# ipilter/RayTracerTest

Measured on AMD Instinct MI355X. Metric: Mray/s at 1920x1080x16spp, higher is better.
Workload: dtype f32

## Files before the change

### include/rt_mi355x.h

```cpp
#ifndef RT_MI355X_H
#define RT_MI355X_H

#include <stddef.h>
#include <stdint.h>

#ifdef __cplusplus
extern "C" {
#endif

#define RT_OK              0
#define RT_ERR_INVALID     1
#define RT_ERR_NO_DEVICE   2
#define RT_ERR_HIP         3
#define RT_ERR_STATE       4

#define RT_MATH_FMA        0u
#define RT_MATH_STRICT     1u

#define RT_FLAG_NO_FILTER  1u
#define RT_FLAG_NO_BINNING 2u

#define RT_FLAG_NEAREST_HIT 4u

#define RT_FLAG_NO_MACRO_BINS 16u
// ... 44 lines not shown
void rt_tracer_stop(rt_tracer* t);
int  rt_tracer_resize(rt_tracer* t, const uint32_t size[2]);
void rt_tracer_set_camera_parameters(rt_tracer* t, float fov, float focalLength, float aperture);
void rt_tracer_rotate_camera(rt_tracer* t, const float angles[2]);
int  rt_tracer_upload_scene(rt_tracer* t, const rt_float4* hostData, size_t count);
int  rt_tracer_upload_scene_edges(rt_tracer* t, const rt_float4* hostData, size_t count);
float rt_pack_normal(const float n[3]);
void  rt_unpack_normal(float packed, float n[3]);
void rt_tracer_set_update_callback(rt_tracer* t, rt_callback_fn fn, void* user);
void rt_tracer_set_finished_callback(rt_tracer* t, rt_callback_fn fn, void* user);


int  rt_tracer_wait(rt_tracer* t);
int  rt_tracer_set_seed(rt_tracer* t, uint64_t seed);
int  rt_tracer_upload_spheres(rt_tracer* t, const rt_float4* spheres, size_t count);
int  rt_tracer_trace_enqueue(rt_tracer* t, uint32_t iterationCount, uint32_t samplesPerIteration);
int  rt_tracer_trace_enqueue_n(rt_tracer* t, uint32_t iterationCount, uint32_t samplesPerIteration, uint32_t n_steps);
int  rt_tracer_sync(rt_tracer* t);
int  rt_tracer_launch(rt_tracer* t, uint32_t samples, int clear_first, int emit_image);
int  rt_tracer_launch_iterations(rt_tracer* t, uint32_t samples, uint32_t iterations, int clear_first, int emit_image);
int  rt_tracer_fused_iterations(rt_tracer* t, uint32_t samples);
int  rt_tracer_set_list_reuse(rt_tracer* t, int across_traces);
int  rt_tracer_set_image_mirror(rt_tracer* t, void* device_visible_image);
int  rt_tracer_kernel_time(rt_tracer* t, double* total_ms, uint64_t* launches, int reset_after);
int  rt_tracer_launch_time(rt_tracer* t, double* total_ms, uint64_t* launches, int reset_after);
int  rt_tracer_trace_stats(rt_tracer* t, uint32_t samples, uint64_t out[16]);
int  rt_tracer_read_buffer(rt_tracer* t, int which, void* dst, size_t bytes);
int  rt_tracer_copy_buffer_to_device(rt_tracer* t, int which, void* dst_device, size_t bytes);
int  rt_tracer_copy_buffer_to_device_async(rt_tracer* t, int which, void* dst_device, size_t bytes);
void* rt_tracer_stream(rt_tracer* t);
void* rt_tracer_stream_b(rt_tracer* t);
void* rt_tracer_device_pointer(rt_tracer* t, int which);
size_t rt_tracer_buffer_bytes(rt_tracer* t, int which);
int  rt_tracer_info(rt_tracer* t, uint32_t out[8]);
const char* rt_tracer_last_error(rt_tracer* t);
const char* rt_last_error(void);
int  rt_device_count(void);
const char* rt_version(void);

typedef struct rt_hit { float t, u, v; int32_t prim; } rt_hit;
#define RT_PRIM_NONE (-1)
int  rt_tracer_intersect(rt_tracer* t, const float* rays, size_t n, rt_hit* hits);
int  rt_tracer_intersect_device(rt_tracer* t, const float* rays, size_t n, rt_hit* hits, void* stream);
int  rt_tracer_pick(rt_tracer* t, const uint32_t* pixels, size_t n, rt_hit* hits, float* rays);
int  rt_tracer_focus_at(rt_tracer* t, uint32_t x, uint32_t y, float* focal_length);

#define RT_QUERY_SCAN 0u
#define RT_QUERY_BVH  1u
int  rt_tracer_set_query_accel(rt_tracer* t, uint32_t mode);
int  rt_tracer_query_accel_info(rt_tracer* t, uint64_t out[8]);

int  rt_tracer_occluded(rt_tracer* t, const float* segs, size_t n, uint8_t* occluded);
int  rt_tracer_occluded_device(rt_tracer* t, const float* segs, size_t n, uint8_t* occluded, void* stream);


int  rt_tracer_create_multi(const uint32_t imageSize[2], const float cameraPosition[3],
                            const float cameraAngles[2], float fov, float focalLength, float aperture,
                            const rt_options* options, const int32_t* devices, uint32_t n_bands,
                            rt_tracer** out);
int  rt_group_unique_id(uint8_t id[RT_GROUP_ID_BYTES]);
int  rt_tracer_join_group(rt_tracer* t, uint32_t n_ranks, uint32_t rank, const uint8_t id[RT_GROUP_ID_BYTES]);
int  rt_tracer_leave_group(rt_tracer* t);
int  rt_tracer_join_group_bands(rt_tracer* t, uint32_t n_ranks, uint32_t rank, const uint8_t id[RT_GROUP_ID_BYTES],
                                const uint32_t* row_begin);
int  rt_balance_rows(uint32_t n_bands, const uint32_t* row_begin, const double* cost, uint32_t granule,
                     uint32_t* new_row_begin);
int  rt_tracer_rebalance(rt_tracer* t);
int  rt_tracer_set_band(rt_tracer* t, uint32_t row_begin, uint32_t rows);
int  rt_tracer_gather_time(rt_tracer* t, double* total_ms, uint64_t* gathers, int reset_after);
int  rt_tracer_gather_only(rt_tracer* t);
int  rt_tracer_group_info(rt_tracer* t, char* json, size_t capacity);
int  rt_tracer_band_count(rt_tracer* t);
int  rt_tracer_band_info(rt_tracer* t, uint32_t band, uint32_t out[4]);

int rt_dbg_hit_triangle(int device, uint32_t math_mode, uint32_t n, const float* rays,
                        const float* tris, int eps_mode, int32_t* hit, float* tuv, float* normal,
                        float* point);
int rt_dbg_sincos(int device, uint32_t n, const float* x, float* s, float* c);
int rt_dbg_trace_occupancy(int device, int samples_in_flight, uint32_t lds_bytes);
int rt_dbg_valu_peak(int device, double* lane_fma_per_s, double* clock_ghz);
int rt_dbg_check_midrange(int device, uint64_t out[4]);
int rt_dbg_wave_list_counts(rt_tracer* t, int half, uint32_t* dst, size_t capacity_tiles, uint32_t* n_tiles, uint32_t* capacity_per_tile);
int rt_dbg_read_tile_lists(rt_tracer* t, uint32_t* dst, size_t capacity_words, uint32_t* words_per_tile);
int rt_dbg_focal_boxes(rt_tracer* t, float curv_scale, float* boxes, size_t boxes_capacity, float* focal, size_t focal_capacity);
int rt_dbg_classify(rt_tracer* t, uint32_t level, uint32_t forms, uint32_t slack_milli, const uint32_t* regions, uint32_t n_regions,
                    float* out, size_t capacity_floats);
int rt_dbg_bvh_build(const rt_float4* rows, size_t count, int edges_layout, void* nodes, size_t node_capacity_bytes,
                     void* leaf_records, size_t leaf_capacity_bytes, uint64_t info[8]);
int rt_dbg_query_accel_slack(rt_tracer* t, uint32_t slack_milli);
int rt_dbg_uniform(int device, uint32_t n, uint32_t m, uint32_t* states, float* out);
int rt_dbg_get_ray(rt_tracer* t, uint32_t n, const uint32_t* pixels, uint32_t* states, float* rays);
void rt_dbg_rng_init_host(uint64_t seed, uint64_t subsequence, uint32_t state[6]);

#ifdef __cplusplus
}
#endif
#endif
```

### raytracertest_amd/api.py

```python
import ctypes as C
import os
import threading
import weakref

import numpy as np

_HERE = os.path.dirname(os.path.abspath(__file__))
_LIB_PATH = os.environ.get("RT_MI355X_LIB") or os.path.join(_HERE, "lib", "librt_mi355x.so")

MATH_FMA, MATH_STRICT = 0, 1
FLAG_NO_FILTER = 1
FLAG_NO_BINNING = 2
FLAG_NEAREST_HIT = 4
FLAG_SMOOTH_NORMALS = 8
FLAG_NO_MACRO_BINS = 16
FLAG_NO_SUPER_BINS = 64
FLAG_NO_SURE_HIT = 32
BUF_RENDER, BUF_COUNTS, BUF_IMAGE, BUF_RNG, BUF_FRAME = 0, 1, 2, 3, 4
GROUP_ID_BYTES = 128
TRANSPORT_RCCL, TRANSPORT_PEER = 0, 1

ABI_SYMBOLS = [
    "rt_tracer_create", "rt_tracer_create_ex", "rt_tracer_destroy", "rt_tracer_trace",
    "rt_tracer_stop", "rt_tracer_resize", "rt_tracer_set_camera_parameters",
    "rt_tracer_rotate_camera", "rt_tracer_upload_scene", "rt_tracer_set_update_callback",
    "rt_tracer_set_finished_callback", "rt_tracer_wait", "rt_tracer_set_seed",
    "rt_tracer_upload_spheres", "rt_tracer_trace_enqueue", "rt_tracer_trace_enqueue_n", "rt_tracer_sync", "rt_tracer_trace_stats", "rt_tracer_launch", "rt_tracer_launch_iterations", "rt_tracer_fused_iterations", "rt_tracer_set_image_mirror", "rt_tracer_set_list_reuse", "rt_tracer_stream_b", "rt_tracer_upload_scene_edges", "rt_pack_normal",
    "rt_unpack_normal",
    "rt_tracer_kernel_time", "rt_tracer_launch_time", "rt_tracer_read_buffer", "rt_tracer_copy_buffer_to_device", "rt_tracer_copy_buffer_to_device_async",
    "rt_tracer_stream",
    "rt_tracer_device_pointer", "rt_tracer_buffer_bytes", "rt_tracer_info",
    "rt_tracer_last_error", "rt_last_error", "rt_device_count", "rt_version",
    "rt_dbg_hit_triangle", "rt_dbg_sincos", "rt_dbg_valu_peak", "rt_dbg_check_midrange", "rt_dbg_trace_occupancy", "rt_dbg_uniform", "rt_dbg_get_ray",
    "rt_dbg_rng_init_host",
    "rt_tracer_create_multi", "rt_group_unique_id", "rt_tracer_join_group", "rt_tracer_leave_group",
    "rt_tracer_gather_time", "rt_tracer_band_count", "rt_tracer_band_info",
    "rt_tracer_join_group_bands", "rt_balance_rows", "rt_tracer_rebalance", "rt_tracer_set_band", "rt_dbg_read_tile_lists", "rt_dbg_wave_list_counts", "rt_dbg_focal_boxes", "rt_dbg_classify",
    "rt_tracer_gather_only", "rt_tracer_group_info",
    "rt_tracer_intersect", "rt_tracer_intersect_device", "rt_tracer_pick", "rt_tracer_focus_at",
    "rt_tracer_occluded", "rt_tracer_occluded_device",
    "rt_tracer_set_query_accel", "rt_tracer_query_accel_info", "rt_dbg_bvh_build", "rt_dbg_query_accel_slack",
]


class RtError(RuntimeError):
    pass


PRIM_NONE = -1
QUERY_SCAN, QUERY_BVH = 0, 1
BVH_NODE_DTYPE = np.dtype([("lo", np.float32, (3, 4)), ("hi", np.float32, (3, 4)), ("child", np.uint32, 4), ("cmax", np.float32, 4)])
BVH_RECORD_DTYPE = np.dtype([("e2", np.float32, 3), ("e1", np.float32, 3), ("v0", np.float32, 3), ("index", np.uint32), ("pad", np.uint32, 2)])
BVH_EMPTY, BVH_LEAF = 0xFFFFFFFF, 0x80000000
_ACCEL_KEYS = ("mode", "valid", "nodes", "leaves", "depth", "always_tested", "build_us", "device_bytes")


def bvh_build(rows, edges=False):
    L = load_library()
    r = np.ascontiguousarray(rows, np.float32).reshape(-1, 4)
    info = (C.c_uint64 * 8)()
    if L.rt_dbg_bvh_build(r.ctypes.data, r.shape[0], int(bool(edges)), None, 0, None, 0, info) != 0:
        raise RtError("rt_dbg_bvh_build: " + L.rt_last_error().decode())
    nodes = np.zeros(int(info[2]), BVH_NODE_DTYPE)
    recs = np.zeros(r.shape[0] // 3, BVH_RECORD_DTYPE)
    if L.rt_dbg_bvh_build(r.ctypes.data, r.shape[0], int(bool(edges)), nodes.ctypes.data, max(nodes.nbytes, 1), recs.ctypes.data,
                          max(recs.nbytes, 1), info) != 0:
        raise RtError("rt_dbg_bvh_build: " + L.rt_last_error().decode())
    d = dict(zip(_ACCEL_KEYS, (int(x) for x in info)))
    d["depth_bound"] = d.pop("mode")
    return nodes, recs, d
HIT_DTYPE = np.dtype([("t", np.float32), ("u", np.float32), ("v", np.float32), ("prim", np.int32)])


class Options(C.Structure):
    _fields_ = [("struct_size", C.c_uint32), ("device", C.c_int32), ("full_height", C.c_uint32),
                ("row_begin", C.c_uint32), ("use_time_seed", C.c_uint32), ("math_mode", C.c_uint32),
                ("seed", C.c_uint64), ("flags", C.c_uint32), ("samples_in_flight", C.c_uint32),
                ("lds_chunk", C.c_uint32), ("bin_list", C.c_uint32), ("transport", C.c_uint32)]


CALLBACK = C.CFUNCTYPE(None, C.POINTER(C.c_uint32), C.c_size_t, C.c_void_p)

_lib = None
_lib_lock = threading.Lock()


def library_path():
    return _LIB_PATH


def _share_hip_runtime_with_torch():
    if os.environ.get("RT_MI355X_HIP_RUNTIME", "") == "system":
        return None
    try:
        import importlib.util
        spec = importlib.util.find_spec("torch")
        if spec is None or not spec.submodule_search_locations:
            return None
        cand = os.path.join(list(spec.submodule_search_locations)[0], "lib", "libamdhip64.so")
        if os.path.exists(cand):
            C.CDLL(cand, mode=C.RTLD_GLOBAL)
            return cand
    except (ImportError, OSError, ValueError):
        pass
    return None


HIP_RUNTIME = None


def load_library():
    global _lib, HIP_RUNTIME
    with _lib_lock:
        if _lib is not None:
            return _lib
        if not os.path.exists(_LIB_PATH):
            raise RtError("HIP extension not built: %s is missing (run `python -m raytracertest_amd.build` "
                          "or __graft_entry__.build()); there is no CPU fallback" % _LIB_PATH)
        HIP_RUNTIME = _share_hip_runtime_with_torch()
        L = C.CDLL(_LIB_PATH)
        vp, u32p, f32p = C.c_void_p, C.POINTER(C.c_uint32), C.POINTER(C.c_float)
        L.rt_tracer_create.argtypes = [u32p, f32p, f32p, C.c_float, C.c_float, C.c_float, C.POINTER(vp)]
        L.rt_tracer_create_ex.argtypes = [u32p, f32p, f32p, C.c_float, C.c_float, C.c_float,
                                          C.POINTER(Options), C.POINTER(vp)]
        L.rt_tracer_destroy.argtypes = [vp]
        L.rt_tracer_destroy.restype = None
        L.rt_tracer_trace.argtypes = [vp, C.c_uint32, C.c_uint32, C.c_uint32]
        L.rt_tracer_stop.argtypes = [vp]
        L.rt_tracer_stop.restype = None
        L.rt_tracer_resize.argtypes = [vp, u32p]
        L.rt_tracer_set_camera_parameters.argtypes = [vp, C.c_float, C.c_float, C.c_float]
        L.rt_tracer_set_camera_parameters.restype = None
        L.rt_tracer_rotate_camera.argtypes = [vp, f32p]
        L.rt_tracer_rotate_camera.restype = None
        L.rt_tracer_upload_scene.argtypes = [vp, vp, C.c_size_t]
        L.rt_tracer_upload_scene_edges.argtypes = [vp, vp, C.c_size_t]
        L.rt_pack_normal.argtypes = [f32p]
        L.rt_pack_normal.restype = C.c_float
        L.rt_unpack_normal.argtypes = [C.c_float, f32p]
        L.rt_unpack_normal.restype = None
        L.rt_tracer_set_update_callback.argtypes = [vp, CALLBACK, vp]
        L.rt_tracer_set_update_callback.restype = None
        L.rt_tracer_set_finished_callback.argtypes = [vp, CALLBACK, vp]
        L.rt_tracer_set_finished_callback.restype = None
        L.rt_tracer_wait.argtypes = [vp]
        L.rt_tracer_set_seed.argtypes = [vp, C.c_uint64]
        L.rt_tracer_upload_spheres.argtypes = [vp, vp, C.c_size_t]
        L.rt_tracer_trace_enqueue.argtypes = [vp, C.c_uint32, C.c_uint32]
        L.rt_tracer_trace_enqueue_n.argtypes = [vp, C.c_uint32, C.c_uint32, C.c_uint32]
        L.rt_tracer_sync.argtypes = [vp]
        L.rt_tracer_launch.argtypes = [vp, C.c_uint32, C.c_int, C.c_int]
        L.rt_tracer_launch_iterations.argtypes = [vp, C.c_uint32, C.c_uint32, C.c_int, C.c_int]
        L.rt_tracer_fused_iterations.argtypes = [vp, C.c_uint32]
        L.rt_tracer_set_image_mirror.argtypes = [vp, vp]
        L.rt_tracer_set_list_reuse.argtypes = [vp, C.c_int]
        L.rt_tracer_trace_stats.argtypes = [vp, C.c_uint32, C.POINTER(C.c_uint64)]
        L.rt_tracer_kernel_time.argtypes = [vp, C.POINTER(C.c_double), C.POINTER(C.c_uint64), C.c_int]
        L.rt_tracer_launch_time.argtypes = [vp, C.POINTER(C.c_double), C.POINTER(C.c_uint64), C.c_int]
        L.rt_tracer_read_buffer.argtypes = [vp, C.c_int, vp, C.c_size_t]
        L.rt_tracer_copy_buffer_to_device.argtypes = [vp, C.c_int, vp, C.c_size_t]
        L.rt_tracer_copy_buffer_to_device_async.argtypes = [vp, C.c_int, vp, C.c_size_t]
        L.rt_tracer_stream.argtypes = [vp]
        L.rt_tracer_stream.restype = vp
        L.rt_tracer_stream_b.argtypes = [vp]
        L.rt_tracer_stream_b.restype = vp
        L.rt_tracer_device_pointer.argtypes = [vp, C.c_int]
        L.rt_tracer_device_pointer.restype = vp
        L.rt_tracer_buffer_bytes.argtypes = [vp, C.c_int]
        L.rt_tracer_buffer_bytes.restype = C.c_size_t
        L.rt_tracer_info.argtypes = [vp, u32p]
        L.rt_tracer_last_error.argtypes = [vp]
        L.rt_tracer_last_error.restype = C.c_char_p
        L.rt_last_error.restype = C.c_char_p
        L.rt_device_count.restype = C.c_int
        L.rt_version.restype = C.c_char_p
        L.rt_dbg_hit_triangle.argtypes = [C.c_int, C.c_uint32, C.c_uint32, f32p, f32p, C.c_int,
                                          C.POINTER(C.c_int32), f32p, f32p, f32p]
        L.rt_dbg_sincos.argtypes = [C.c_int, C.c_uint32, f32p, f32p, f32p]
        L.rt_dbg_uniform.argtypes = [C.c_int, C.c_uint32, C.c_uint32, u32p, f32p]
        L.rt_dbg_valu_peak.argtypes = [C.c_int, C.POINTER(C.c_double), C.POINTER(C.c_double)]
        L.rt_dbg_trace_occupancy.argtypes = [C.c_int, C.c_int, C.c_uint32]
        L.rt_dbg_get_ray.argtypes = [vp, C.c_uint32, u32p, u32p, f32p]
        L.rt_dbg_rng_init_host.argtypes = [C.c_uint64, C.c_uint64, u32p]
        L.rt_dbg_rng_init_host.restype = None
        L.rt_tracer_create_multi.argtypes = [u32p, f32p, f32p, C.c_float, C.c_float, C.c_float, C.POINTER(Options),
                                             C.POINTER(C.c_int32), C.c_uint32, C.POINTER(vp)]
        L.rt_group_unique_id.argtypes = [C.c_char_p]
        L.rt_tracer_join_group.argtypes = [vp, C.c_uint32, C.c_uint32, C.c_char_p]
        L.rt_tracer_leave_group.argtypes = [vp]
        L.rt_tracer_gather_time.argtypes = [vp, C.POINTER(C.c_double), C.POINTER(C.c_uint64), C.c_int]
        L.rt_tracer_band_count.argtypes = [vp]
        L.rt_tracer_band_info.argtypes = [vp, C.c_uint32, u32p]
        L.rt_tracer_join_group_bands.argtypes = [vp, C.c_uint32, C.c_uint32, C.c_char_p, u32p]
        L.rt_balance_rows.argtypes = [C.c_uint32, u32p, C.POINTER(C.c_double), C.c_uint32, u32p]
        L.rt_tracer_rebalance.argtypes = [vp]
        L.rt_tracer_set_band.argtypes = [vp, C.c_uint32, C.c_uint32]
        L.rt_dbg_read_tile_lists.argtypes = [vp, u32p, C.c_size_t, u32p]
        L.rt_dbg_wave_list_counts.argtypes = [vp, C.c_int, u32p, C.c_size_t, u32p, u32p]
        L.rt_dbg_focal_boxes.argtypes = [vp, C.c_float, f32p, C.c_size_t, f32p, C.c_size_t]
        L.rt_tracer_gather_only.argtypes = [vp]
        L.rt_tracer_group_info.argtypes = [vp, C.c_char_p, C.c_size_t]
        L.rt_dbg_classify.argtypes = [vp, C.c_uint32, C.c_uint32, C.c_uint32, u32p, C.c_uint32, f32p, C.c_size_t]
        L.rt_tracer_intersect.argtypes = [vp, vp, C.c_size_t, vp]
        L.rt_tracer_intersect_device.argtypes = [vp, vp, C.c_size_t, vp, vp]
        L.rt_tracer_pick.argtypes = [vp, vp, C.c_size_t, vp, vp]
        L.rt_tracer_focus_at.argtypes = [vp, C.c_uint32, C.c_uint32, f32p]
        L.rt_tracer_occluded.argtypes = [vp, vp, C.c_size_t, vp]
        L.rt_tracer_occluded_device.argtypes = [vp, vp, C.c_size_t, vp, vp]
        L.rt_tracer_set_query_accel.argtypes = [vp, C.c_uint32]
        L.rt_tracer_query_accel_info.argtypes = [vp, C.POINTER(C.c_uint64)]
        L.rt_dbg_query_accel_slack.argtypes = [vp, C.c_uint32]
        L.rt_dbg_bvh_build.argtypes = [vp, C.c_size_t, C.c_int, vp, C.c_size_t, vp, C.c_size_t, C.POINTER(C.c_uint64)]
        _lib = L
        return _lib


def device_count():
    return int(load_library().rt_device_count())


def balance_rows(row_begin, cost, granule=8):
    b = np.ascontiguousarray(row_begin, np.uint32)
    c = np.ascontiguousarray(cost, np.float64)
    out = np.zeros_like(b)
    rc = load_library().rt_balance_rows(c.size, _u32p(b), c.ctypes.data_as(C.POINTER(C.c_double)), granule, _u32p(out))
    if rc != 0:
        raise RtError("rt_balance_rows: invalid partition")
    return [int(x) for x in out]


def group_unique_id():
    buf = C.create_string_buffer(GROUP_ID_BYTES)
    rc = load_library().rt_group_unique_id(buf)
    if rc != 0:
        raise RtError("rt_group_unique_id failed (%d): %s" % (rc, load_library().rt_last_error().decode()))
    return buf.raw


def _f32p(a):
    return a.ctypes.data_as(C.POINTER(C.c_float))


def _u32p(a):
    return a.ctypes.data_as(C.POINTER(C.c_uint32))


class RayTracer:

    def __init__(self, imageSize, cameraPosition=(0.0, 0.0, 0.0), cameraAngles=(0.0, 0.0), fov=70.0,
                 focalLength=10.0, aperture=4.0, *, seed=None, device=0, math_mode=MATH_FMA,
                 full_height=0, row_begin=0, no_filter=False, no_binning=False, nearest_hit=False, smooth_normals=False, no_macro_bins=False, no_super_bins=False, samples_in_flight=0,
                 lds_chunk=0, bin_list=0, devices=None, no_sure_hit=False, transport="rccl"):
        self._lib = load_library()
        self._h = C.c_void_p()
        self._cbs = {}
        self._retired = []
        size = np.array(imageSize, np.uint32)
        opt = Options()
        opt.struct_size = C.sizeof(Options)
        opt.device = device
        opt.full_height, opt.row_begin = full_height, row_begin
        opt.use_time_seed = 1 if seed is None else 0
        opt.seed = 0 if seed is None else int(seed)
        opt.math_mode = math_mode
        opt.flags = ((FLAG_NO_FILTER if no_filter else 0) | (FLAG_NO_BINNING if no_binning else 0) |
                     (FLAG_NEAREST_HIT if nearest_hit else 0) | (FLAG_SMOOTH_NORMALS if smooth_normals else 0) | (FLAG_NO_MACRO_BINS if no_macro_bins else 0) | (FLAG_NO_SUPER_BINS if no_super_bins else 0) |
                     (FLAG_NO_SURE_HIT if no_sure_hit else 0))
        opt.samples_in_flight, opt.lds_chunk, opt.bin_list = samples_in_flight, lds_chunk, bin_list
        opt.transport = {"rccl": TRANSPORT_RCCL, "peer": TRANSPORT_PEER}[transport]
        if devices is not None:
            devs = np.ascontiguousarray(devices, np.int32)
            rc = self._lib.rt_tracer_create_multi(_u32p(size), _f32p(np.array(cameraPosition, np.float32)),
                                                  _f32p(np.array(cameraAngles, np.float32)), fov, focalLength, aperture,
                                                  C.byref(opt), devs.ctypes.data_as(C.POINTER(C.c_int32)), devs.size,
                                                  C.byref(self._h))
        else:
            rc = self._lib.rt_tracer_create_ex(_u32p(size), _f32p(np.array(cameraPosition, np.float32)),
                                               _f32p(np.array(cameraAngles, np.float32)), fov, focalLength,
                                               aperture, C.byref(opt), C.byref(self._h))
        if rc != 0 or not self._h:
            raise RtError("rt_tracer_create failed (%d): %s" % (rc, self._lib.rt_last_error().decode()))
# ... 117 lines not shown
        return np.ascontiguousarray(np.moveaxis(planes, 0, -1))

    def JoinGroup(self, n_ranks, rank, unique_id=None, row_begin=None):
        if row_begin is None:
            self._check(self._lib.rt_tracer_join_group(self._h, n_ranks, rank, unique_id))
        else:
            b = np.ascontiguousarray(row_begin, np.uint32)
            self._check(self._lib.rt_tracer_join_group_bands(self._h, n_ranks, rank, unique_id, _u32p(b)))

    def SetBand(self, row_begin, rows):
        self._check(self._lib.rt_tracer_set_band(self._h, row_begin, rows))
        self.rows = int(rows)

    def Rebalance(self):
        self._check(self._lib.rt_tracer_rebalance(self._h))

    def LeaveGroup(self):
        self._check(self._lib.rt_tracer_leave_group(self._h))

    def Frame(self):
        return self._read(BUF_FRAME, np.uint32, (self.full_height, self.width))

    def GatherTime(self, reset=True):
        ms, n = C.c_double(), C.c_uint64()
        self._lib.rt_tracer_gather_time(self._h, C.byref(ms), C.byref(n), 1 if reset else 0)
        return ms.value, n.value

    def GatherOnly(self):
        self._check(self._lib.rt_tracer_gather_only(self._h))

    def GroupInfo(self):
        import json
        buf = C.create_string_buffer(8192)
        self._check(self._lib.rt_tracer_group_info(self._h, buf, len(buf)))
        return json.loads(buf.value.decode())

    def Bands(self):
        out = []
        for k in range(int(self._lib.rt_tracer_band_count(self._h))):
            v = np.zeros(4, np.uint32)
            self._check(self._lib.rt_tracer_band_info(self._h, k, _u32p(v)))
            out.append({"device": int(v[0]), "row0": int(v[1]), "rows": int(v[2]), "rank": int(v[3])})
        return out

    def DevicePointer(self, which):
        return self._lib.rt_tracer_device_pointer(self._h, which)

    def CopyToDevice(self, which, dst_ptr, nbytes):
        self._check(self._lib.rt_tracer_copy_buffer_to_device(self._h, which, dst_ptr, nbytes))

    def CopyToDeviceAsync(self, which, dst_ptr, nbytes):
        self._check(self._lib.rt_tracer_copy_buffer_to_device_async(self._h, which, dst_ptr, nbytes))

    def Stream(self):
        return int(self._lib.rt_tracer_stream(self._h) or 0)

    def StreamB(self):
        return int(self._lib.rt_tracer_stream_b(self._h) or 0)

    def Info(self):
        out = np.zeros(8, np.uint32)
        self._lib.rt_tracer_info(self._h, _u32p(out))
        keys = ("samples_in_flight", "lds_chunk", "lds_bytes", "grid_x", "grid_y", "n_tris", "n_spheres", "device")
        return dict(zip(keys, (int(v) for v in out)))

    def LastError(self):
        return self._lib.rt_tracer_last_error(self._h).decode()

    def DebugTileLists(self):
        bx, by = (self.width + 31) // 32, (self.rows + 7) // 8
        wpt = np.zeros(1, np.uint32)
        buf = np.zeros(bx * (by + 1) * 4 * 1025, np.uint32)
        self._check(self._lib.rt_dbg_read_tile_lists(self._h, _u32p(buf), buf.size, _u32p(wpt)))
        w = int(wpt[0])
        words = buf[:bx * by * 4 * w].reshape(by, bx * 4, w)[:, :, 0]
        return (words & 0x3FF).astype(np.int32), ((words >> 10) & 0x3FF).astype(np.int32), (words >> 31).astype(bool)

    def DebugWaveListCounts(self, half=0):
        n, cap = np.zeros(1, np.uint32), np.zeros(1, np.uint32)
        buf = np.zeros(((self.width + 31) // 32) * ((self.rows + 7) // 8 + 1) * 4, np.uint32)
        self._check(self._lib.rt_dbg_wave_list_counts(self._h, half, _u32p(buf), buf.size, _u32p(n), _u32p(cap)))
        return buf[:int(n[0])].copy(), int(cap[0])

    def DebugTileListWords(self):
        bx, by = (self.width + 31) // 32, (self.rows + 7) // 8
        wpt = np.zeros(1, np.uint32)
        buf = np.zeros(bx * (by + 1) * 4 * 1025, np.uint32)
        self._check(self._lib.rt_dbg_read_tile_lists(self._h, _u32p(buf), buf.size, _u32p(wpt)))
        w = int(wpt[0])
        return buf[:bx * by * 4 * w].reshape(by, bx * 4, w).copy()

    def DebugFocalBoxes(self, curv_scale=1.0):
        bx, by = (self.width + 31) // 32, (self.rows + 7) // 8
        boxes = np.zeros((by, bx * 4, 8), np.float32)
        focal = np.zeros((self.rows, self.width, 3), np.float32)
        self._check(self._lib.rt_dbg_focal_boxes(self._h, float(curv_scale), _f32p(boxes), boxes.size, _f32p(focal), focal.size))
        return boxes, focal

    def DebugClassify(self, regions, level=0, forms=False, slack_milli=1000):
        reg = np.ascontiguousarray(regions, np.uint32).reshape(-1, 2)
        n_tris = self.Info()["n_tris"]
        per = 16 + n_tris * (32 if forms else 12)
        out = np.zeros((reg.shape[0], per), np.float32)
        self._check(self._lib.rt_dbg_classify(self._h, level, 1 if forms else 0, slack_milli, _u32p(reg), reg.shape[0], _f32p(out), out.size))
        return out[:, :16], out[:, 16:].reshape(reg.shape[0], n_tris, 32 if forms else 12)

    def Intersect(self, rays):
        if type(rays).__module__.startswith("torch"):
            return self._intersect_tensor(rays)
        r = np.ascontiguousarray(rays, np.float32).reshape(-1, 6)
        hits = np.zeros(r.shape[0], HIT_DTYPE)
        self._check(self._lib.rt_tracer_intersect(self._h, r.ctypes.data, r.shape[0], hits.ctypes.data))
        return hits

    def _intersect_tensor(self, rays):
        import torch
        if rays.dtype != torch.float32 or rays.dim() != 2 or rays.shape[1] != 6 or not rays.is_contiguous():
            raise ValueError("Intersect: expected a contiguous (n, 6) float32 tensor")
        dev = self.Bands()[0]["device"]
        if rays.device.type != "cuda" or rays.device.index != dev:
            raise ValueError("Intersect: the rays are on %s, the tracer on cuda:%d" % (rays.device, dev))
        hits = torch.empty((rays.shape[0], 4), dtype=torch.float32, device=rays.device)
        stream = torch.cuda.current_stream(rays.device).cuda_stream
        self._check(self._lib.rt_tracer_intersect_device(self._h, rays.data_ptr(), rays.shape[0], hits.data_ptr(),
                                                         C.c_void_p(stream)))
        return hits

    def Pick(self, pixels, return_rays=False):
        pix = np.ascontiguousarray(pixels, np.uint32).reshape(-1, 2)
        hits = np.zeros(pix.shape[0], HIT_DTYPE)
        rays = np.zeros((pix.shape[0], 6), np.float32) if return_rays else None
        self._check(self._lib.rt_tracer_pick(self._h, pix.ctypes.data, pix.shape[0], hits.ctypes.data,
                                             None if rays is None else rays.ctypes.data))
        return (hits, rays) if return_rays else hits

    def FocusAt(self, x, y):
        f = C.c_float()
        self._check(self._lib.rt_tracer_focus_at(self._h, x, y, C.byref(f)))
        return np.float32(f.value)

    def Occluded(self, segs):
        if type(segs).__module__.startswith("torch"):
            return self._occluded_tensor(segs)
        s = np.asarray(segs, np.float32)
        if s.ndim == 0 or s.shape[-1] != 8:
            raise ValueError("Occluded: expected (n, 8) float32 segments, got shape %s" % (s.shape,))
        s = np.ascontiguousarray(s).reshape(-1, 8)
        out = np.zeros(s.shape[0], np.uint8)
        self._check(self._lib.rt_tracer_occluded(self._h, s.ctypes.data, s.shape[0], out.ctypes.data))
        return out.view(np.bool_)

    def _occluded_tensor(self, segs):
        import torch
        if segs.dtype != torch.float32 or segs.dim() != 2 or segs.shape[1] != 8 or not segs.is_contiguous():
            raise ValueError("Occluded: expected a contiguous (n, 8) float32 tensor")
        dev = self.Bands()[0]["device"]
        if segs.device.type != "cuda" or segs.device.index != dev:
            raise ValueError("Occluded: the segments are on %s, the tracer on cuda:%d" % (segs.device, dev))
        out = torch.empty((segs.shape[0],), dtype=torch.uint8, device=segs.device)
        stream = torch.cuda.current_stream(segs.device).cuda_stream
        self._check(self._lib.rt_tracer_occluded_device(self._h, segs.data_ptr(), segs.shape[0], out.data_ptr(),
                                                        C.c_void_p(stream)))
        return out

    def Visible(self, a, b, tmin=0.0, tmax=1.0):
        a = np.asarray(a, np.float32).reshape(-1, 3)
# ... 126 lines not shown
```

### raytracertest_amd/csrc/rt_debug.hip

```cpp
#include "rt_tracer.hpp"

using namespace rtr;

template <class F>
static int on_device(int device, F&& f) {
  const int rc = require_device(device);
  if (rc != RT_OK) return rc;
  return guarded(nullptr, [&] { HIP_CHECK(hipSetDevice(device)); f(); });
}

template <class F>
static int on_tracer(rt_tracer* t, F&& f) { return exclusive(t, [&] { t->use_device(); f(); }); }

extern "C" {

int rt_dbg_hit_triangle(int device, uint32_t math_mode, uint32_t n, const float* rays, const float* tris,
                        int eps_mode, int32_t* hit, float* tuv, float* normal, float* point) {
  return on_device(device, [&] {
    DevArray<float> dr(n * 6), dt(n * 9), duv(n * 3), dn(n * 3), dp(n * 3);
    DevArray<int> dh(n);
    HIP_CHECK(hipMemcpy(dr.get(), rays, n * 6 * sizeof(float), hipMemcpyHostToDevice));
    HIP_CHECK(hipMemcpy(dt.get(), tris, n * 9 * sizeof(float), hipMemcpyHostToDevice));
    HIP_CHECK(rtk::launch_dbg_hit_triangle(math_mode != RT_MATH_STRICT, n, dr.get(), dt.get(), eps_mode, dh.get(), duv.get(),
                                           dn.get(), dp.get(), nullptr));
    HIP_CHECK(hipDeviceSynchronize());
    HIP_CHECK(hipMemcpy(hit, dh.get(), n * sizeof(int), hipMemcpyDeviceToHost));
    HIP_CHECK(hipMemcpy(tuv, duv.get(), n * 3 * sizeof(float), hipMemcpyDeviceToHost));
    HIP_CHECK(hipMemcpy(normal, dn.get(), n * 3 * sizeof(float), hipMemcpyDeviceToHost));
    HIP_CHECK(hipMemcpy(point, dp.get(), n * 3 * sizeof(float), hipMemcpyDeviceToHost));
  });
}

int rt_dbg_check_midrange(int device, uint64_t out[4]) {
  if (!out) return RT_ERR_INVALID;
  return on_device(device, [&] {
    DevArray<unsigned long long> d(4);
    HIP_CHECK(hipMemset(d.get(), 0, 4 * sizeof(unsigned long long)));
    HIP_CHECK(rtk::launch_dbg_check_midrange(d.get(), nullptr));
    HIP_CHECK(hipDeviceSynchronize());
    HIP_CHECK(hipMemcpy(out, d.get(), 4 * sizeof(uint64_t), hipMemcpyDeviceToHost));
  });
}

int rt_dbg_valu_peak(int device, double* lane_fma_per_s, double* clock_ghz) {
  return on_device(device, [&] {
    hipDeviceProp_t prop;
    HIP_CHECK(hipGetDeviceProperties(&prop, device));
    const uint32_t blocks = static_cast<uint32_t>(prop.multiProcessorCount) * 8u;
    const int iters = 20000;
    DevArray<float> out(static_cast<size_t>(blocks) * 256);
    DevArray<unsigned long long> clk(2);
    const Event e0 = Event::timing(), e1 = Event::timing();
    HIP_CHECK(rtk::launch_dbg_valu_peak(blocks, iters, out.get(), clk.get(), nullptr));
    HIP_CHECK(hipEventRecord(e0, nullptr));
    HIP_CHECK(rtk::launch_dbg_valu_peak(blocks, iters, out.get(), clk.get(), nullptr));
    HIP_CHECK(hipEventRecord(e1, nullptr));
    HIP_CHECK(hipEventSynchronize(e1));
    float ms = 0.0f;
    HIP_CHECK(hipEventElapsedTime(&ms, e0, e1));
    unsigned long long c[2];
    HIP_CHECK(hipMemcpy(c, clk.get(), sizeof c, hipMemcpyDeviceToHost));
    if (lane_fma_per_s) *lane_fma_per_s = static_cast<double>(blocks) * 256.0 * iters * 8.0 / (ms * 1e-3);
    if (clock_ghz) *clock_ghz = c[1] ? static_cast<double>(c[0]) / static_cast<double>(c[1]) * 0.1 : 0.0;
  });
}

#ifdef RT_TIMELINE
int rt_dbg_trace_timeline(rt_tracer* t, uint32_t samples, unsigned long long* out, size_t capacity_words) {
  if (!t || !out) return RT_ERR_INVALID;
  return on_tracer(t, [&] {
    const size_t words = static_cast<size_t>((t->W + 31u) / 32u) * ((t->rows + 7u) / 8u) * 4u * 16u;
    if (words > capacity_words) throw HipFail{fmt("timeline needs %zu words", words)};
    DevArray<unsigned long long> buf(words);
    HIP_CHECK(hipMemsetAsync(buf.get(), 0, words * sizeof(unsigned long long), t->main_stream()));
    rtk::TraceParams p = t->params(samples);
    p.flags = rtk::TRACE_ZERO_ACC | rtk::TRACE_EMIT_IMAGE | t->mode_flags(p);
    p.image = t->d_image.get();
    p.timeline = buf.get();
    t->launch_instrumented(p, samples);
    HIP_CHECK(hipMemcpy(out, buf.get(), words * sizeof(unsigned long long), hipMemcpyDeviceToHost));
  });
}
#endif

int rt_dbg_read_tile_lists(rt_tracer* t, uint32_t* dst, size_t capacity_words, uint32_t* words_per_tile) {
  if (!t || t->mg || !dst) return RT_ERR_INVALID;
  return on_tracer(t, [&] {
    HIP_CHECK(hipStreamSynchronize(t->main_stream()));
    t->sync_list_stream();
    if (!t->lists.now() || !t->lists.key) throw HipFail{"no tile lists (small scenes build them ahead of their first trace launch)"};
    const size_t n = t->lists.words() < capacity_words ? t->lists.words() : capacity_words;
    HIP_CHECK(hipMemcpy(dst, t->lists.now(), n * sizeof(uint32_t), hipMemcpyDeviceToHost));
    if (words_per_tile) *words_per_tile = 1u + t->lists.key->bin_list;
  });
}

int rt_dbg_wave_list_counts(rt_tracer* t, int half, uint32_t* dst, size_t capacity_tiles, uint32_t* n_tiles, uint32_t* capacity_per_tile) {
  if (!t || t->mg || !dst || half < 0 || half > 1) return RT_ERR_INVALID;
  return on_tracer(t, [&] {
    HIP_CHECK(hipStreamSynchronize(t->main_stream()));
    const HalfLists& h = t->half_lists[half];
    if (!h.wave.get() || !h.wave_valid) throw HipFail{"no wave lists (dense scenes build them ahead of their first trace launch)"};
    const size_t n = h.wave_tiles < capacity_tiles ? h.wave_tiles : capacity_tiles;
    HIP_CHECK(hipMemcpy2D(dst, sizeof(uint32_t), h.wave.get(), static_cast<size_t>(1u + h.wave_cap) * 64u, sizeof(uint32_t), n, hipMemcpyDeviceToHost));
    if (n_tiles) *n_tiles = static_cast<uint32_t>(h.wave_tiles);
    if (capacity_per_tile) *capacity_per_tile = h.wave_cap;
  });
}

int rt_dbg_trace_occupancy(int device, int samples_in_flight, uint32_t lds_bytes) {
  if (require_device(device) != RT_OK) return -1;
  if (hipSetDevice(device) != hipSuccess) return -1;
  return rtk::trace_occupancy(samples_in_flight, lds_bytes);
}

int rt_dbg_sincos(int device, uint32_t n, const float* x, float* s, float* c) {
  return on_device(device, [&] {
    DevArray<float> dx(n), ds(n), dc(n);
    HIP_CHECK(hipMemcpy(dx.get(), x, n * sizeof(float), hipMemcpyHostToDevice));
    HIP_CHECK(rtk::launch_dbg_sincos(n, dx.get(), ds.get(), dc.get(), nullptr));
    HIP_CHECK(hipDeviceSynchronize());
    HIP_CHECK(hipMemcpy(s, ds.get(), n * sizeof(float), hipMemcpyDeviceToHost));
    HIP_CHECK(hipMemcpy(c, dc.get(), n * sizeof(float), hipMemcpyDeviceToHost));
  });
}

int rt_dbg_uniform(int device, uint32_t n, uint32_t m, uint32_t* states, float* out) {
  return on_device(device, [&] {
    DevArray<uint32_t> ds(n * 6);
    DevArray<float> dout(static_cast<size_t>(n) * m);
    HIP_CHECK(hipMemcpy(ds.get(), states, n * 6 * sizeof(uint32_t), hipMemcpyHostToDevice));
    HIP_CHECK(rtk::launch_dbg_uniform(n, m, ds.get(), dout.get(), nullptr));
    HIP_CHECK(hipDeviceSynchronize());
    HIP_CHECK(hipMemcpy(states, ds.get(), n * 6 * sizeof(uint32_t), hipMemcpyDeviceToHost));
    HIP_CHECK(hipMemcpy(out, dout.get(), static_cast<size_t>(n) * m * sizeof(float), hipMemcpyDeviceToHost));
  });
}

int rt_dbg_get_ray(rt_tracer* t, uint32_t n, const uint32_t* pixels, uint32_t* states, float* rays) {
  if (!t) return RT_ERR_INVALID;
  if (t->mg) { multi_push_camera(t); return rt_dbg_get_ray(t->mg->bands[0], n, pixels, states, rays); }
  return guarded(t, [&] {
    t->use_device();
    rtk::TraceParams p = t->params(1);
    DevArray<uint32_t> dpix(n * 2), ds(n * 6);
    DevArray<float> dr(n * 6);
    HIP_CHECK(hipMemcpy(dpix.get(), pixels, n * 2 * sizeof(uint32_t), hipMemcpyHostToDevice));
    HIP_CHECK(hipMemcpy(ds.get(), states, n * 6 * sizeof(uint32_t), hipMemcpyHostToDevice));
    HIP_CHECK(rtk::launch_dbg_get_ray(t->fma, p, n, dpix.get(), ds.get(), dr.get(), t->main_stream()));
    HIP_CHECK(hipStreamSynchronize(t->main_stream()));
    HIP_CHECK(hipMemcpy(states, ds.get(), n * 6 * sizeof(uint32_t), hipMemcpyDeviceToHost));
    HIP_CHECK(hipMemcpy(rays, dr.get(), n * 6 * sizeof(float), hipMemcpyDeviceToHost));
  });
}

int rt_dbg_focal_boxes(rt_tracer* t, float curv_scale, float* boxes, size_t boxes_capacity, float* focal, size_t focal_capacity) {
  if (!t || t->mg || !boxes || !focal) return RT_ERR_INVALID;
  return on_tracer(t, [&] {
    rtk::TraceParams p = t->params(1);
    if (p.tile_curv > 0.0f) p.tile_curv = std::max(p.tile_curv * curv_scale, 1e-30f);
    const size_t tiles = static_cast<size_t>((t->W + 31u) / 32u) * ((t->rows + 7u) / 8u) * 4u;
    const size_t nb = tiles * 8u, nf = static_cast<size_t>(t->npix()) * 3u;
    if (nb > boxes_capacity || nf > focal_capacity) throw HipFail{fmt("focal boxes need %zu + %zu floats", nb, nf)};
    DevArray<float> db(nb), df(nf);
    HIP_CHECK(hipMemsetAsync(db.get(), 0, nb * sizeof(float), t->main_stream()));
    HIP_CHECK(rtk::launch_dbg_focal_boxes(t->fma, p, db.get(), df.get(), t->main_stream()));
    HIP_CHECK(hipStreamSynchronize(t->main_stream()));
    HIP_CHECK(hipMemcpy(boxes, db.get(), nb * sizeof(float), hipMemcpyDeviceToHost));
    HIP_CHECK(hipMemcpy(focal, df.get(), nf * sizeof(float), hipMemcpyDeviceToHost));
  });
}

int rt_dbg_classify(rt_tracer* t, uint32_t level, uint32_t forms, uint32_t slack_milli, const uint32_t* regions, uint32_t n_regions,
                    float* out, size_t capacity_floats) {
  if (!t || t->mg || !regions || !out || level > 4u) return RT_ERR_INVALID;
  return on_tracer(t, [&] {
// ... 25 lines not shown
```

### raytracertest_amd/csrc/rt_kernels.hpp

```cpp
#pragma once
#include <hip/hip_runtime.h>
#include <stdint.h>

namespace rtk {

constexpr uint32_t kSuperChunk = 1024u, kSuperMaxChunks = 64u;

struct TraceParams {
  float4*   render;
  uint32_t* rng;
  uint32_t  weyl, count;
  uint32_t  W, H;
  uint32_t  row0, rows;
  uint32_t  npix;
  uint32_t  samples;
  float     cam[12];
  float     half_height, aspect, focal, aperture;
  float     tile_curv, tile_round;
  const float4* tri_a;
  const float*  tri_b;
  const float4* tri_color;
  uint32_t  n_tris;
  const float4* spheres;
  uint32_t  n_spheres;
  uint32_t  chunk;
  uint32_t  bin_list;
  uint32_t  block_list;
  unsigned long long* stats;
  uint32_t* image;
  const float4* tri_n;
#ifdef RT_TIMELINE
  unsigned long long* timeline;
#endif
  uint32_t* image_host;
  uint32_t  pretest_on;
  uint32_t  iters;
  uint32_t* macro_lists;
  uint32_t  macro_cap, macro_w, macro_h, macro_nx;
  uint32_t* super_lists;
  uint32_t  super_chunks, super_f, super_nx;
  float*    macro_bounds;
  uint32_t* tile_lists;
  uint32_t  row_il, row_phase;
  uint32_t* half_cost;
  uint32_t  cost_split_brow;
  const float4* sure_table;
  uint32_t* wave_lists;
  uint32_t  wave_cap;
  uint32_t  flags;
};

constexpr uint32_t TRACE_ZERO_ACC = 1u;
constexpr uint32_t TRACE_EMIT_IMAGE = 2u;
constexpr uint32_t TRACE_NEAREST_HIT = 4u;
constexpr uint32_t TRACE_PRETEST = 32u;
constexpr uint32_t TRACE_NO_SURE_HIT = 64u;

enum class TracePath : uint32_t {
  FullScan,
  SmallLists,
  Classify,
  ClassifyForms,
  DenseLists,
};

hipError_t launch_rng_init(uint32_t* rng, uint32_t npix, uint32_t p0, const uint32_t seeded[6],
                           const uint32_t* jump, const uint32_t* win, hipStream_t st);
hipError_t launch_prep_triangles(bool fma, bool edges, const float4* verts, uint32_t n, float4* tri_a, float* tri_b,
                                 float4* color, float4* normals, hipStream_t st);
uint32_t trace_lds_bytes(const TraceParams& p, TracePath path);
hipError_t launch_trace(const TraceParams& p, bool fma, bool filter, TracePath path, int K, hipStream_t st);
int trace_occupancy(int K, size_t lds);
hipError_t launch_convert(const float4* render, uint32_t count, uint32_t* image, uint32_t npix, hipStream_t st);

uint32_t query_lds_bytes(uint32_t n_tris, int K);
hipError_t launch_query(const TraceParams& p, bool fma, int K, uint32_t n, const float* rays, const uint32_t* pixels,
                        float* rays_out, float4* hits, hipStream_t st);

#define RT_BVH_RHO 0.00390625f

struct BvhParams {
  const float4* nodes;
  const float4* records;
  uint32_t n_nodes;
  uint32_t n_leaf_records;
  uint32_t n_always;
  uint32_t stack_cap;
  float rho;
};
uint32_t query_bvh_lds_bytes(uint32_t stack_cap);
hipError_t launch_query_bvh(const TraceParams& p, const BvhParams& b, bool fma, uint32_t n, const float* rays, const uint32_t* pixels,
                            float* rays_out, float4* hits, hipStream_t st);

uint32_t occluded_lds_bytes(uint32_t n_tris);
hipError_t launch_occluded(const TraceParams& p, bool fma, int K, uint32_t n, const float* segs, uint8_t* occluded, hipStream_t st);
uint32_t occluded_bvh_lds_bytes(uint32_t stack_cap);
hipError_t launch_occluded_bvh(const TraceParams& p, const BvhParams& b, bool fma, uint32_t n, const float* segs, uint8_t* occluded,
                               hipStream_t st);

hipError_t launch_dbg_hit_triangle(bool fma, uint32_t n, const float* rays, const float* tris, int eps_mode,
                                   int* hit, float* tuv, float* normal, float* point, hipStream_t st);
bool trace_can_fuse(TracePath path, bool filter);
hipError_t launch_macro_bin(const TraceParams& p, bool fma, hipStream_t st);
hipError_t launch_super_bin(const TraceParams& p, bool fma, hipStream_t st);
hipError_t launch_wave_lists(const TraceParams& p, bool fma, hipStream_t st);
hipError_t launch_delay(uint32_t us, hipStream_t st);
hipError_t launch_publish_half_cost(uint32_t* half_cost, unsigned long long* host_word, hipStream_t st);
hipError_t launch_sure_table(const float4* colors, uint32_t n_tris, uint32_t samples, float4* out, hipStream_t st);
hipError_t launch_tile_lists(const TraceParams& p, bool fma, hipStream_t st);
hipError_t launch_dbg_check_midrange(unsigned long long* out, hipStream_t st);
hipError_t launch_dbg_focal_boxes(bool fma, const TraceParams& p, float* boxes, float* focal, hipStream_t st);
hipError_t launch_dbg_classify(bool fma, bool forms, uint32_t slack_milli, const TraceParams& p, uint32_t level, uint32_t n_regions,
                               const uint32_t* regions, float* out, hipStream_t st);
hipError_t launch_dbg_valu_peak(uint32_t blocks, int iters, float* out, unsigned long long* clk, hipStream_t st);
hipError_t launch_dbg_sincos(uint32_t n, const float* x, float* s, float* c, hipStream_t st);
hipError_t launch_dbg_uniform(uint32_t n, uint32_t m, uint32_t* states, float* out, hipStream_t st);
hipError_t launch_dbg_get_ray(bool fma, const TraceParams& p, uint32_t n, const uint32_t* pixels,
                              uint32_t* states, float* rays, hipStream_t st);

}
```

### raytracertest_amd/csrc/rt_lists.hpp

```cpp
#pragma once
#include "rt_classify.hpp"

namespace rtk {

template <bool FMA, int WAVES>
__device__ __forceinline__ FocalBounds rect_focal_bounds(const TraceParams& p, uint32_t x0, uint32_t y0, uint32_t rw, uint32_t rh, float (*s_box)[8]) {
  const uint32_t lane = threadIdx.x & 63u, wave = threadIdx.x >> 6;
  const uint32_t x1 = (x0 + rw < p.W) ? x0 + rw : p.W;
  const uint32_t y1 = (y0 + rh < p.rows) ? y0 + rh : p.rows;
  const uint32_t w = x1 - x0, count_px = w * (y1 - y0);
  float lo[3] = {FLT_MAX, FLT_MAX, FLT_MAX}, hi[3] = {-FLT_MAX, -FLT_MAX, -FLT_MAX};
  bool finite = true;
  for (uint32_t i = threadIdx.x; i < count_px; i += 64u * WAVES) {
    const uint32_t px = x0 + i % w, ly = y0 + i / w;
    V3 po, pd;
    pinhole<FMA>(p, px, p.row0 + ly, po, pd);
    const V3 f = focal_point<FMA>(p, pd);
    const float fl[3] = {f.x, f.y, f.z};
#pragma unroll
    for (int c = 0; c < 3; ++c) {
      finite = finite && (__builtin_fabsf(fl[c]) <= FLT_MAX);
      lo[c] = fminf(lo[c], fl[c]);
      hi[c] = fmaxf(hi[c], fl[c]);
    }
// ... 150 lines not shown
__device__ __forceinline__ float group_min(float v) {
  RT_ROW_REDUCE(fminf, v)
#pragma unroll
  for (int off = G / 2; off >= 16; off >>= 1) v = fminf(v, __shfl_xor(v, off, 64));
  return v;
}
#undef RT_ROW_REDUCE

template <bool FMA, int G, class SL>
__device__ __forceinline__ FocalBounds group_focal_bounds(const TraceParams& p, uint32_t x0, uint32_t y0, bool in_image, uint32_t gl, uint32_t gbase) {
  constexpr uint32_t T = 64u / G;
  const bool full = in_image && x0 + 8u <= p.W && y0 + 8u <= p.rows;
  FocalBounds b;
  const bool corners = p.tile_curv > 0.0f && full;
  const unsigned long long need_range = __builtin_amdgcn_ballot_w64(in_image && !corners);
  {
    const uint32_t cx = x0 + ((gl & 1u) ? 7u : 0u), cy = y0 + ((gl & 2u) ? 7u : 0u);
    V3 po, pd;
    pinhole<FMA>(p, cx < p.W ? cx : 0u, p.row0 + (cy < p.rows ? cy : 0u), po, pd);
    const V3 f = focal_point<FMA>(p, pd);
    const float fl[3] = {f.x, f.y, f.z};
    const float dev = p.tile_curv + RT_SLK(4e-6f) * p.tile_round;
    bool finite = true;
#pragma unroll
    for (int i = 0; i < 3; ++i) {
      const float c0 = __shfl(fl[i], static_cast<int>(gbase), 64), c1 = __shfl(fl[i], static_cast<int>(gbase + 1u), 64);
      const float c2 = __shfl(fl[i], static_cast<int>(gbase + 2u), 64), c3 = __shfl(fl[i], static_cast<int>(gbase + 3u), 64);
      b.lo[i] = fminf(fminf(c0, c1), fminf(c2, c3)) - dev;
      b.hi[i] = fmaxf(fmaxf(c0, c1), fmaxf(c2, c3)) + dev;
      finite = finite && (__builtin_fabsf(b.lo[i]) <= FLT_MAX) && (__builtin_fabsf(b.hi[i]) <= FLT_MAX);
    }
    b.ok = finite; b.any = true;
  }
  if (need_range != 0ull) {
    float lo[3] = {FLT_MAX, FLT_MAX, FLT_MAX}, hi[3] = {-FLT_MAX, -FLT_MAX, -FLT_MAX};
    bool finite = true, any = false;
#pragma unroll
    for (uint32_t i = 0; i < T; ++i) {
      const uint32_t pi = gl + i * G;
      const uint32_t px = x0 + (pi & 7u), py = y0 + (pi >> 3);
      const bool inside = in_image && px < p.W && py < p.rows;
      V3 po, pd;
      pinhole<FMA>(p, inside ? px : 0u, p.row0 + (inside ? py : 0u), po, pd);
      const V3 f = focal_point<FMA>(p, pd);
      const float fl[3] = {f.x, f.y, f.z};
#pragma unroll
      for (int c = 0; c < 3; ++c) {
        if (inside) { lo[c] = fminf(lo[c], fl[c]); hi[c] = fmaxf(hi[c], fl[c]); finite = finite && (__builtin_fabsf(fl[c]) <= FLT_MAX); }
      }
      any = any || inside;
    }
    const unsigned long long gmask = G == 64 ? ~0ull : (0xFFFFFFFFull << gbase);
    const bool g_ok = (__builtin_amdgcn_ballot_w64(!finite) & gmask) == 0ull;
    const bool g_any = (__builtin_amdgcn_ballot_w64(any) & gmask) != 0ull;
#pragma unroll
    for (int c = 0; c < 3; ++c) { lo[c] = group_min<G>(lo[c]); hi[c] = group_max<G>(hi[c]); }
    if (!corners) {
#pragma unroll
      for (int c = 0; c < 3; ++c) { b.lo[c] = lo[c]; b.hi[c] = hi[c]; }
      b.ok = g_ok; b.any = g_any;
    }
  }
  return b;
}

template <bool FMA, int G, class SL = SlackProduct>
__global__ __launch_bounds__(256, 5) void tile_lists_kernel(const TraceParams p) {
  static_assert(G == 32 || G == 64, "lanes per tile");
  constexpr uint32_t T = 64u / G;
  const uint32_t lane = threadIdx.x & 63u, wave = threadIdx.x >> 6;
  const uint32_t gl = lane & (G - 1u), gbase = lane & ~(G - 1u);
  const uint32_t gx = (p.W + 31u) / 32u, gy = (p.rows + 7u) / 8u;
  const uint32_t slots = gx * gy * 4u;
  const uint32_t slot = (blockIdx.x * 4u + wave) * T + lane / G;
  const bool live = slot < slots;
  const uint32_t sl = live ? slot : 0u;
  const uint32_t x0 = ((sl / 4u) % gx) * 32u + (sl % 4u) * 8u, y0 = ((sl / 4u) / gx) * 8u;
  const bool in_image = live && x0 < p.W;

  const FocalBounds b = group_focal_bounds<FMA, G, SL>(p, x0, y0, in_image, gl, gbase);
  const TileFamily fam = make_family<SL>(p, b);

  uint32_t* const saved = p.tile_lists + static_cast<size_t>(sl) * (1u + p.bin_list);
  const uint32_t n = p.n_tris;
  uint32_t count = 0;
  const float NEG = -__builtin_inff();
  bool haveA = false;
  float Q = NEG, M1 = NEG, M2 = NEG;
  uint32_t A = 0, I1 = 0xFFFFFFFFu;
  for (uint32_t base = 0; base < n; base += G) {
    const uint32_t tri = base + gl;
    const bool valid = in_image && tri < n;
    const uint32_t ti = tri < n ? tri : n - 1u;
    const float4 A0 = p.tri_a[2u * ti], A1 = p.tri_a[2u * ti + 1u];
    const float bz = p.tri_b[ti];
    bool keep = valid, sure = false;
    float q[2] = {0.0f, 0.0f};
    if (fam.usable) {
      const bool miss = tile_misses_triangle<false, true, SL>(fam, {A1.z, A1.w, bz}, {A0.w, A1.x, A1.y}, {A0.x, A0.y, A0.z}, nullptr, &sure, q);
      keep = valid && !miss;
    } else {
      sure = false;
    }
    const unsigned long long m = __builtin_amdgcn_ballot_w64(keep);
    const unsigned long long gm = G == 64 ? m : ((m >> gbase) & 0xFFFFFFFFull);
    const uint32_t pos = count + static_cast<uint32_t>(__builtin_popcountll(gm & ((1ull << gl) - 1ull)));
    if (keep) saved[1u + pos] = tri;
    count += static_cast<uint32_t>(__builtin_popcountll(gm));
    const bool cand = keep && sure && fam.usable;
    const float Qs = group_max<G>(cand ? q[0] : NEG);
    const unsigned long long bm = __builtin_amdgcn_ballot_w64(cand && q[0] == Qs);
    const unsigned long long gbm = G == 64 ? bm : ((bm >> gbase) & 0xFFFFFFFFull);
    if (gbm != 0ull && (!haveA || Qs > Q)) { haveA = true; Q = Qs; A = base + static_cast<uint32_t>(__builtin_ctzll(gbm)); }
    const float qh = keep ? ((q[1] == q[1]) ? q[1] : __builtin_inff()) : NEG;
    if (n <= G) {
      const uint32_t la = gbm != 0ull ? static_cast<uint32_t>(__builtin_ctzll(gbm)) : 0xFFFFFFFFu;
      M1 = group_max<G>((keep && gl != la) ? qh : NEG);
      I1 = 0xFFFFFFFEu;
      break;
    }
    const float m1s = group_max<G>(qh);
    const unsigned long long tm = __builtin_amdgcn_ballot_w64(keep && qh == m1s);
    const unsigned long long gtm = G == 64 ? tm : ((tm >> gbase) & 0xFFFFFFFFull);
    const uint32_t l1 = gtm != 0ull ? static_cast<uint32_t>(__builtin_ctzll(gtm)) : 0xFFFFFFFFu;
    const float m2s = group_max<G>((keep && gl != l1) ? qh : NEG);
    if (gtm != 0ull) {
      if (m1s > M1) { M2 = fmaxf(M1, m2s); M1 = m1s; I1 = base + l1; }
      else { M2 = fmaxf(M2, m1s); }
    }
  }
  bool sure_one = false;
  if (haveA) {
    const float R = (I1 == A) ? M2 : M1;
    sure_one = count <= 1u || (R < Q - 1e-4f * (__builtin_fabsf(R) + __builtin_fabsf(Q)));
  }
  if (live && gl == 0u) saved[0] = count | (A << 10) | (sure_one ? 0x80000000u : 0u);
}

template <class SL>
__device__ __forceinline__ float tile_dev(const TraceParams& p) { return p.tile_curv + RT_SLK(4e-6f) * p.tile_round; }

__device__ __forceinline__ void region_corner_pixel(const TraceParams& p, uint32_t rx, uint32_t ry, uint32_t tile, uint32_t corner,
                                                    uint32_t& px, uint32_t& py, bool& valid) {
  const uint32_t x0 = rx * 32u + (tile & 3u) * 8u, y0 = (ry * 2u + (tile >> 2)) * 8u;
  valid = x0 < p.W && y0 < p.rows;
  const uint32_t x1 = (x0 + 7u < p.W) ? x0 + 7u : p.W - 1u, y1 = (y0 + 7u < p.rows) ? y0 + 7u : p.rows - 1u;
  px = valid ? ((corner & 1u) ? x1 : x0) : 0u;
  py = valid ? ((corner & 2u) ? y1 : y0) : 0u;
}

template <bool FMA, class SL, bool PACK = false>
__device__ __forceinline__ void region_focal_bounds(const TraceParams& p, uint32_t rx, uint32_t ry, uint32_t lane,
                                                    FocalBounds& tile_b, FocalBounds& region_b) {
  const uint32_t l32 = lane & 31u;
  uint32_t px, py;
  bool valid;
  region_corner_pixel(p, rx, ry, l32 >> 2, l32 & 3u, px, py, valid);
  V3 po, pd;
  pinhole<FMA>(p, px, p.row0 + py, po, pd);
  const V3 f = focal_point<FMA>(p, pd);
  const float fl[3] = {f.x, f.y, f.z};
  const float dev = tile_dev<SL>(p);
  bool fin = true;
  float rlo[3], rhi[3];
#pragma unroll
  for (int i = 0; i < 3; ++i) {
    float lo = fl[i], hi = fl[i];
    lo = fminf(lo, dpp_f<0xB1>(lo)); lo = fminf(lo, dpp_f<0x4E>(lo));
    hi = fmaxf(hi, dpp_f<0xB1>(hi)); hi = fmaxf(hi, dpp_f<0x4E>(hi));
    tile_b.lo[i] = lo - dev;
    tile_b.hi[i] = hi + dev;
    fin = fin && (__builtin_fabsf(tile_b.lo[i]) <= FLT_MAX) && (__builtin_fabsf(tile_b.hi[i]) <= FLT_MAX) && (fl[i] == fl[i]);
    rlo[i] = valid ? tile_b.lo[i] : FLT_MAX;
    rhi[i] = valid ? tile_b.hi[i] : -FLT_MAX;
  }
  const unsigned long long badm = __builtin_amdgcn_ballot_w64(!fin);
  const uint32_t quad_bad = (static_cast<uint32_t>(badm >> (lane & (PACK ? 60u : 28u))) & 0xFu);
  tile_b.ok = quad_bad == 0u;
  tile_b.any = valid;
  const unsigned long long vm = __builtin_amdgcn_ballot_w64(valid);
  const uint32_t hs = PACK ? (lane & 32u) : 0u;
  region_b.any = ((vm >> hs) & 0xFFFFFFFFull) != 0ull;
  region_b.ok = (((badm & vm) >> hs) & 0xFFFFFFFFull) == 0ull;
#pragma unroll
  for (int i = 0; i < 3; ++i) {
    region_b.lo[i] = group_min<32>(rlo[i]);
    region_b.hi[i] = group_max<32>(rhi[i]);
  }
}


template <int G>
__device__ __forceinline__ float max_group(float v) {
  v = fmaxf(v, dpp_f<0xB1>(v));
  v = fmaxf(v, dpp_f<0x4E>(v));
  if constexpr (G == 8) v = fmaxf(v, dpp_f<0x141>(v));
  return v;
}

template <class SL, int G2>
__device__ __forceinline__ void region_level2(const TraceParams& p, uint32_t lane, const FocalBounds& mine, const uint32_t* cand, uint32_t cnt,
                                              uint32_t cnt_max, uint32_t tslot, bool slot_live, bool lower) {
  constexpr uint32_t GM = (1u << G2) - 1u;
  const uint32_t j = lane & (G2 - 1u), gsh = lane & ~static_cast<uint32_t>(G2 - 1);
  const bool tile_valid = mine.any;
  const TileFamily fam = make_family<SL>(p, mine);
  uint32_t* const saved = p.tile_lists + static_cast<size_t>(tile_valid ? tslot : 0u) * (1u + p.bin_list);
  const float NEG = -__builtin_inff();
  uint32_t count = 0;
  bool haveA = false;
  float Q = NEG, M1 = NEG, M2 = NEG;
  uint32_t A = 0, I1 = 0xFFFFFFFFu;
  const bool one_pass = cnt_max <= static_cast<uint32_t>(G2);
  bool others_ok = true;
  for (uint32_t c0 = 0; c0 < cnt_max; c0 += G2) {
    const bool has = tile_valid && c0 + j < cnt;
    const uint32_t tri = (c0 + j < cnt) ? cand[c0 + j] : 0u;
    const float4 A0 = p.tri_a[2u * tri], A1 = p.tri_a[2u * tri + 1u];
    const float bz = p.tri_b[tri];
    bool keep = has, sure = false;
    float q[2] = {0.0f, 0.0f};
    float pr[9] = {0.0f, 0.0f, 0.0f, 0.0f, 0.0f, 0.0f, 0.0f, 0.0f, 0.0f};
    if (fam.usable) {
      const bool miss = tile_misses_triangle<false, true, SL>(fam, {A1.z, A1.w, bz}, {A0.w, A1.x, A1.y}, {A0.x, A0.y, A0.z}, nullptr, &sure, q,
                                                              nullptr, pr);
      keep = has && !miss;
    }
    const uint32_t gm = static_cast<uint32_t>(__builtin_amdgcn_ballot_w64(keep) >> gsh) & GM;
    const uint32_t pos = count + static_cast<uint32_t>(__builtin_popcount(gm & ((1u << j) - 1u)));
    if (keep) saved[1u + pos] = tri;
    count += static_cast<uint32_t>(__builtin_popcount(gm));
    const bool cd = keep && sure && fam.usable;
    const float Qs = max_group<G2>(cd ? q[0] : NEG);
    const uint32_t gbm = static_cast<uint32_t>(__builtin_amdgcn_ballot_w64(cd && q[0] == Qs) >> gsh) & GM;
    if (gbm != 0u && (!haveA || Qs > Q)) { haveA = true; Q = Qs; A = cand[c0 + static_cast<uint32_t>(__builtin_ctz(gbm))]; }
    const float qh = keep ? ((q[1] == q[1]) ? q[1] : __builtin_inff()) : NEG;
    if (one_pass) {
      const uint32_t la = gbm != 0u ? static_cast<uint32_t>(__builtin_ctz(gbm)) : 0xFFFFFFFFu;
      bool lane_ok = !keep || j == la || (gbm != 0u && qh < Qs - 1e-4f * (__builtin_fabsf(qh) + __builtin_fabsf(Qs)));
      const bool need = gbm != 0u && !lane_ok;
      if (__builtin_amdgcn_ballot_w64(need) != 0ull) {
        float pa[9];
        const int src = static_cast<int>(gsh + (la & (G2 - 1u)));
#pragma unroll
        for (int i = 0; i < 9; ++i) pa[i] = __shfl(pr[i], src, 64);
        lane_ok = lane_ok || (need && pair_farther<SL>(fam, pa, pr));
      }
      others_ok = (static_cast<uint32_t>(__builtin_amdgcn_ballot_w64(!lane_ok) >> gsh) & GM) == 0u;
    }
    const float m1s = max_group<G2>(qh);
    const uint32_t gtm = static_cast<uint32_t>(__builtin_amdgcn_ballot_w64(keep && qh == m1s) >> gsh) & GM;
    const uint32_t l1 = gtm != 0u ? static_cast<uint32_t>(__builtin_ctz(gtm)) : 0xFFFFFFFFu;
    const float m2s = max_group<G2>((keep && j != l1) ? qh : NEG);
    if (gtm != 0u) {
      const uint32_t i1s = cand[c0 + l1];
      if (m1s > M1) { M2 = fmaxf(M1, m2s); M1 = m1s; I1 = i1s; }
      else { M2 = fmaxf(M2, m1s); }
    }
  }
  bool sure_one = false;
  if (haveA) {
    const float R = (I1 == A) ? M2 : M1;
    sure_one = count <= 1u || (R < Q - 1e-4f * (__builtin_fabsf(R) + __builtin_fabsf(Q)));
    if (one_pass) sure_one = sure_one || others_ok;
  }
  if (j == 0u) {
    if (tile_valid) saved[0] = count | (A << 10) | (sure_one ? 0x80000000u : 0u);
    else if (slot_live) p.tile_lists[static_cast<size_t>(tslot) * (1u + p.bin_list)] = 0u;
  }
  if (p.half_cost != nullptr) {
    const bool rays = j == 0u && tile_valid && !sure_one;
    const uint32_t nu = static_cast<uint32_t>(__builtin_popcountll(__builtin_amdgcn_ballot_w64(rays && !lower)));
    const uint32_t nl = static_cast<uint32_t>(__builtin_popcountll(__builtin_amdgcn_ballot_w64(rays && lower)));
    if (lane == 0u) {
      if (nu != 0u) atomicAdd(p.half_cost, nu);
      if (nl != 0u) atomicAdd(p.half_cost + 1, nl);
    }
  }
}

template <bool FMA, class SL = SlackProduct>
__global__ __launch_bounds__(256, RT_LISTS_WAVES) void region_lists_kernel(const TraceParams p) {
  __shared__ uint32_t s_cand[4][256];
  const uint32_t lane = threadIdx.x & 63u, wave = threadIdx.x >> 6;
  const uint32_t gx = (p.W + 31u) / 32u, gy = (p.rows + 7u) / 8u, gry = (gy + 1u) / 2u;
  const uint32_t region = blockIdx.x * 4u + wave;
  if (region >= gx * gry) return;
  const uint32_t rx = region % gx, ry = region / gx;
  FocalBounds tb, rb;
  region_focal_bounds<FMA, SL>(p, rx, ry, lane, tb, rb);
  const uint32_t n = p.n_tris;
  uint32_t* const cand = s_cand[wave];

  uint32_t cnt = 0;
  {
    const TileFamily rf = make_family<SL>(p, rb);
    for (uint32_t base = 0; base < n; base += 64u) {
      const uint32_t tri = base + lane;
      const bool valid = tri < n;
      const uint32_t ti = valid ? tri : n - 1u;
      const float4 A0 = p.tri_a[2u * ti], A1 = p.tri_a[2u * ti + 1u];
      const float bz = p.tri_b[ti];
      bool keep = valid;
      if (rf.usable) keep = valid && !tile_misses_triangle<false, false, SL>(rf, {A1.z, A1.w, bz}, {A0.w, A1.x, A1.y}, {A0.x, A0.y, A0.z});
      const unsigned long long m = __builtin_amdgcn_ballot_w64(keep);
      const uint32_t pos = cnt + __builtin_amdgcn_mbcnt_hi(static_cast<uint32_t>(m >> 32), __builtin_amdgcn_mbcnt_lo(static_cast<uint32_t>(m), 0u));
      if (keep) cand[pos] = tri;
      cnt += static_cast<uint32_t>(__builtin_popcountll(m));
    }
    __builtin_amdgcn_fence(__ATOMIC_RELEASE, "wavefront");
    __builtin_amdgcn_wave_barrier();
  }

  const uint32_t t8 = lane >> 3;
  FocalBounds mine;
#pragma unroll
  for (int i = 0; i < 3; ++i) {
    mine.lo[i] = __shfl(tb.lo[i], static_cast<int>(4u * t8), 64);
    mine.hi[i] = __shfl(tb.hi[i], static_cast<int>(4u * t8), 64);
  }
  const unsigned long long okm = __builtin_amdgcn_ballot_w64(tb.ok), anym = __builtin_amdgcn_ballot_w64(tb.any);
  mine.ok = ((okm >> (4u * t8)) & 1ull) != 0ull;
  mine.any = ((anym >> (4u * t8)) & 1ull) != 0ull;
  const uint32_t brow = ry * 2u + (t8 >> 2);
  region_level2<SL, 8>(p, lane, mine, cand, cnt, cnt, (brow * gx + rx) * 4u + (t8 & 3u), brow < gy, brow >= p.cost_split_brow);
}

template <bool FMA, class SL = SlackProduct>
__global__ __launch_bounds__(256, 4) void region_pair_lists_kernel(const TraceParams p) {
  __shared__ uint32_t s_cand[4][2][32];
  const uint32_t lane = threadIdx.x & 63u, wave = threadIdx.x >> 6, half = lane >> 5;
  const uint32_t gx = (p.W + 31u) / 32u, gy = (p.rows + 7u) / 8u, gry = (gy + 1u) / 2u, regions = gx * gry;
  const uint32_t first = (blockIdx.x * 4u + wave) * 2u;
  if (first >= regions) return;
  const bool live = first + half < regions;
  const uint32_t region = live ? first + half : first;
  const uint32_t rx = region % gx, ry = region / gx;
  FocalBounds tb, rb;
  region_focal_bounds<FMA, SL, true>(p, rx, ry, lane, tb, rb);
  const uint32_t n = p.n_tris;
  uint32_t* const cand = s_cand[wave][half];

  uint32_t cnt;
  {
    const TileFamily rf = make_family<SL>(p, rb);
    const uint32_t tri = lane & 31u;
    const bool valid = tri < n;
    const uint32_t ti = valid ? tri : n - 1u;
    const float4 A0 = p.tri_a[2u * ti], A1 = p.tri_a[2u * ti + 1u];
    const float bz = p.tri_b[ti];
    bool keep = valid;
    if (rf.usable) keep = valid && !tile_misses_triangle<false, false, SL>(rf, {A1.z, A1.w, bz}, {A0.w, A1.x, A1.y}, {A0.x, A0.y, A0.z});
// ... 41 lines not shown
```

### raytracertest_amd/csrc/rt_trace.hpp

```cpp
#pragma once
#include "rt_lists.hpp"

namespace rtk {


template <bool FMA, int K, bool FILTER, bool STATS, class GetB>
__device__ __forceinline__ void test_triangle(const float4 A0, const float4 A1, GetB get_v0z, int tri_index,
                                              const V3 (&o)[K], const V3 (&d)[K], float (&best_t)[K],
                                              int (&best_i)[K], bool nearest, bool counted_lane, uint32_t valid_k,
                                              unsigned long long (&st_exit)[4],
                                              unsigned long long (&st_skip)[4]) {
  using M = Math<FMA>;
  const V3 e2 = {A0.x, A0.y, A0.z}, e1 = {A0.w, A1.x, A1.y};

  if constexpr (!FILTER) {
    const V3 v0 = {A1.z, A1.w, get_v0z()};
#pragma unroll
    for (int k = 0; k < K; ++k) {
      float t = 0.0f, u = 0.0f, v = 0.0f;
      int stage;
      const bool h = hit_triangle_exact<FMA>(o[k], d[k], v0, e1, e2, RT_EPS, t, u, v, stage);
      if (h && (nearest ? (t > 0.0f && t < best_t[k]) : best_t[k] < t)) {
        best_t[k] = t;
        best_i[k] = tri_index;
// ... 41 lines not shown
    for (int k = 0; k < K; ++k) {
      qv[k] = M::cross(tv[k], e1);
      V[k] = M::dot(d[k], qv[k]);
      mk[k] &= __builtin_amdgcn_ballot_w64(!(V[k] < tlo[k])) &
               __builtin_amdgcn_ballot_w64(!((U[k] + V[k]) > thi[k]));
      live |= mk[k];
    }
    if (live == 0ull) { if constexpr (STATS) st_skip[2]++; return; }
    if constexpr (STATS) st_skip[3]++;

#pragma unroll
    for (int k = 0; k < K; ++k) {
      if (mk[k] != 0ull) {
        const float inv = 1.0f / det[k];
        const float u = U[k] * inv;
        const float v = V[k] * inv;
        const float t = M::dot(e2, qv[k]) * inv;
        const bool miss = (det[k] < RT_EPS) | (u < 0.0f) | (u > 1.0f) | (v < 0.0f) | (u + v > 1.0f);
        const bool closer = nearest ? ((t > 0.0f) & (t < best_t[k])) : (best_t[k] < t);
        const bool upd = (!miss) & closer;
        best_t[k] = upd ? t : best_t[k];
        best_i[k] = upd ? tri_index : best_i[k];
      }
    }
  }
}


constexpr uint32_t kWaveRec = 16u;
constexpr uint32_t kWaveOverflow = 0xFFFFFFFFu;
template <bool FMA, int K, bool FILTER, bool STATS, TracePath Path, bool FUSE = false>
__global__ __launch_bounds__(256, (Path == TracePath::SmallLists && K == 2) ? 5 : 4) void trace_kernel(const TraceParams p) {
  static_assert(Path != TracePath::DenseLists || (FILTER && !STATS), "lists from HBM: the default dense-scene kernels only");
  using M = Math<FMA>;
  extern __shared__ float4 s_mem[];
  const uint32_t lane = threadIdx.x & 63u;
  const uint32_t wave = threadIdx.x >> 6;
  const uint32_t bx = blockIdx.x;
  uint32_t by = blockIdx.y;
  const uint32_t gxb = gridDim.x;
  if constexpr (Path == TracePath::SmallLists) {
    if (p.row_il != 0u) by = (blockIdx.y / p.row_il) * (2u * p.row_il) + p.row_phase * p.row_il + blockIdx.y % p.row_il;
  }
  const uint32_t px = bx * 32u + wave * 8u + (lane & 7u);
  const uint32_t ly = by * 8u + (lane >> 3);
  const bool inside = px < p.W && ly < p.rows;
  const uint32_t cxp = inside ? px : 0u, cyp = inside ? ly : 0u;
  const size_t pix = static_cast<size_t>(cxp) + static_cast<size_t>(cyp) * p.W;

#ifdef RT_TIMELINE
  const size_t tl_slot = ((static_cast<size_t>(by) * gxb + bx) * 4u + wave) * 16u;
  auto tl_mark = [&](uint32_t i) {
    __builtin_amdgcn_sched_barrier(0);
    if (p.timeline != nullptr && lane == 0u) p.timeline[tl_slot + i] = __builtin_amdgcn_s_memrealtime();
    __builtin_amdgcn_sched_barrier(0);
  };
  if (p.timeline != nullptr && lane == 0u) {
    uint32_t hw, xcc;
    asm volatile("s_getreg_b32 %0, hwreg(HW_REG_HW_ID)" : "=s"(hw));
    asm volatile("s_getreg_b32 %0, hwreg(HW_REG_XCC_ID)" : "=s"(xcc));
    p.timeline[tl_slot + 6] = hw;
    p.timeline[tl_slot + 7] = (static_cast<unsigned long long>(xcc) << 32) | (__builtin_amdgcn_s_memrealtime() & 0xffffffffull);
  }
  tl_mark(0);
#else
  auto tl_mark = [](uint32_t) {};
#endif
  Rng rng;
  auto load_rng = [&] {
    rng.d = p.weyl;
    rng.v0 = p.rng[1 * static_cast<size_t>(p.npix) + pix];
    rng.v1 = p.rng[2 * static_cast<size_t>(p.npix) + pix];
    rng.v2 = p.rng[3 * static_cast<size_t>(p.npix) + pix];
    rng.v3 = p.rng[4 * static_cast<size_t>(p.npix) + pix];
    rng.v4 = p.rng[5 * static_cast<size_t>(p.npix) + pix];
  };
  constexpr bool FORMS = Path == TracePath::ClassifyForms || Path == TracePath::DenseLists;
  constexpr bool RNG_LATE = FORMS;
  constexpr bool THIRD_BLOCK = true, THIRD_WAVE = !FORMS;
  if constexpr (!RNG_LATE) load_rng();


  const bool sure_ok = Path == TracePath::SmallLists && (p.flags & (TRACE_NEAREST_HIT | TRACE_NO_SURE_HIT)) == 0u && p.n_spheres == 0u && p.tri_n == nullptr;
  bool loaded_sure = false;
  uint32_t list_word = 0u;
  if constexpr (Path == TracePath::SmallLists) {
    if (p.tile_lists != nullptr) {
      const size_t slot0 = (static_cast<size_t>(by) * gxb + bx) * 4u + wave;
      list_word = static_cast<uint32_t>(__builtin_amdgcn_readfirstlane(static_cast<int>(p.tile_lists[slot0 * (1u + p.bin_list)])));
      loaded_sure = sure_ok && (list_word >> 31) != 0u;
    }
  }
  V3 po = {0.0f, 0.0f, 0.0f}, pd = {0.0f, 0.0f, 0.0f}, focal = {0.0f, 0.0f, 0.0f};
  if (!loaded_sure) {
    pinhole<FMA>(p, cxp, p.row0 + cyp, po, pd);
    focal = focal_point<FMA>(p, pd);
  }

  const uint32_t n = p.n_tris;
  const bool nearest = (p.flags & TRACE_NEAREST_HIT) != 0u;
  float ax = 0.0f, ay = 0.0f, az = 0.0f;
  unsigned long long st_exit[4] = {0, 0, 0, 0};
  unsigned long long st_skip[4] = {0, 0, 0, 0};
  unsigned long long st_bin[2] = {0, 0};
  unsigned long long st_pre = 0;

  const uint32_t cap = n < p.chunk ? n : p.chunk;
  float4* const sA = s_mem;
  float* const sB = reinterpret_cast<float*>(s_mem + 2u * cap);
  const bool single_chunk = n <= p.chunk;
  if constexpr (Path == TracePath::FullScan) {
    if (single_chunk) {
      for (uint32_t i = threadIdx.x; i < 2u * n; i += 256u) sA[i] = p.tri_a[i];
      for (uint32_t i = threadIdx.x; i < n; i += 256u) sB[i] = p.tri_b[i];
      __syncthreads();
    }
  }

  const uint32_t L = p.bin_list;
  float4* const cA = s_mem + static_cast<size_t>(wave) * (2u * L);
  float* const cB = reinterpret_cast<float*>(s_mem + 4u * 2u * L) + wave * L;
  int* const cI = reinterpret_cast<int*>(s_mem + 4u * 2u * L) + 4u * L + wave * L;
  constexpr bool PRETEST = FORMS;
  const bool pretest = PRETEST && (p.flags & TRACE_PRETEST) != 0u;
  float4* const cP = s_mem + 4u * 2u * L + 2u * L + static_cast<size_t>(wave) * (4u * L);
  const uint32_t list_floats4 = pretest ? (4u * 2u * L + 2u * L + 16u * L) : (4u * 2u * L + 2u * L);
  float* const cC = reinterpret_cast<float*>(s_mem + list_floats4) + wave * (3u * L);

  TileFamily fam;
  bool list_complete = false;
  uint32_t list_count = 0;
  bool sure_hit_tile = false;
  uint32_t sure_winner = 0;
  const uint32_t Lb = p.block_list;
  uint32_t* const bI = reinterpret_cast<uint32_t*>(s_mem + list_floats4);
  uint32_t* const bcnt = bI + Lb;
  float* const bbox = reinterpret_cast<float*>(bcnt + 8);
  uint32_t src_count = n;
  bool src_is_block_list = false;
  const uint32_t* mI = nullptr;
  if constexpr (Path != TracePath::FullScan && Path != TracePath::SmallLists) {
    if (p.macro_lists != nullptr) {
      const uint32_t mt = (blockIdx.y * 8u / p.macro_h) * p.macro_nx + (blockIdx.x * 32u / p.macro_w);
      const uint32_t* const ml = p.macro_lists + static_cast<size_t>(mt) * (p.macro_cap + 1u);
      const uint32_t mc = static_cast<uint32_t>(__builtin_amdgcn_readfirstlane(static_cast<int>(ml[0])));
      if (mc != 0xFFFFFFFFu) { mI = ml + 1; src_count = mc; }
    }
  }
  const uint32_t n_src = src_count;
  if constexpr (Path == TracePath::SmallLists) fam.usable = false;
  bool hbm_overflow = false;
  if constexpr (Path == TracePath::DenseLists) {
    const size_t slot = (static_cast<size_t>(by) * gxb + bx) * 4u + wave;
    const float4* const rec = reinterpret_cast<const float4*>(p.wave_lists) + slot * (1u + p.wave_cap) * (kWaveRec / 4u);
    const float4 hdr = rec[0];
    const uint32_t count = static_cast<uint32_t>(__builtin_amdgcn_readfirstlane(__builtin_bit_cast(int, hdr.x)));
    hbm_overflow = count == kWaveOverflow;
    fam.usable = true;
    fam.fc[0] = uniform(hdr.y); fam.fc[1] = uniform(hdr.z); fam.fc[2] = uniform(hdr.w);
    list_count = hbm_overflow ? 0u : count;
    for (uint32_t e = lane; e < list_count; e += 64u) {
      const float4* const r = rec + (1u + e) * (kWaveRec / 4u);
      const float4 f0 = r[0], f1 = r[1], f2 = r[2], f3 = r[3];
      const uint32_t tri = __builtin_bit_cast(uint32_t, f3.z);
      const float4 a0 = p.tri_a[2u * tri], a1 = p.tri_a[2u * tri + 1u], c0 = p.tri_color[tri];
      const float bz = p.tri_b[tri];
      cP[4u * e] = f0; cP[4u * e + 1u] = f1; cP[4u * e + 2u] = f2; cP[4u * e + 3u] = make_float4(f3.x, f3.y, 0.0f, 0.0f);
      cA[2u * e] = a0; cA[2u * e + 1u] = a1;
      cB[e] = bz;
      cI[e] = static_cast<int>(tri);
      cC[3u * e] = c0.x; cC[3u * e + 1u] = c0.y; cC[3u * e + 2u] = c0.z;
    }
    __builtin_amdgcn_fence(__ATOMIC_RELEASE, "wavefront");
// ... 25 lines not shown
          if (bfam.usable)
            keep = valid && !tile_misses_triangle<false, false, SlackProduct, THIRD_BLOCK>(bfam, {A1.z, A1.w, bz}, {A0.w, A1.x, A1.y}, {A0.x, A0.y, A0.z});
          const unsigned long long m = __builtin_amdgcn_ballot_w64(keep);
          uint32_t* const slot = bcnt + (step & 1u) * 4u;
          if (lane == 0u) slot[wave] = static_cast<uint32_t>(__builtin_popcountll(m));
          __syncthreads();
          const uint32_t c0 = slot[0], c1 = slot[1], c2 = slot[2], c3 = slot[3];
          const uint32_t before = (wave > 0u ? c0 : 0u) + (wave > 1u ? c1 : 0u) + (wave > 2u ? c2 : 0u);
          const uint32_t step_total = c0 + c1 + c2 + c3;
          if (total + step_total > Lb) { overflow = true; break; }
          const uint32_t pos = total + before + __builtin_amdgcn_mbcnt_hi(static_cast<uint32_t>(m >> 32),
                                                                      __builtin_amdgcn_mbcnt_lo(static_cast<uint32_t>(m), 0u));
          if (keep) bI[pos] = tri;
          total += step_total;
        }
        __syncthreads();
        if (!overflow) { src_count = total; src_is_block_list = true; }
      }
    }
  }

  auto classify = [&](uint32_t from, auto with_forms) -> uint32_t {
    constexpr bool WF = decltype(with_forms)::value;
    uint32_t count = 0, base = from;
    while (base < src_count && count < L) {
      const uint32_t e = base + lane;
      const bool valid = e < src_count;
      const uint32_t ei = valid ? e : (src_count - 1u);
      const uint32_t tri = src_is_block_list ? bI[ei] : (mI != nullptr ? mI[ei] : ei);
      const uint32_t ti = tri;
      float4 A0, A1;
      float bz;
      A0 = p.tri_a[2u * ti]; A1 = p.tri_a[2u * ti + 1u];
      bz = p.tri_b[ti];
      bool keep = valid;
      float forms[18] = {0.0f, 0.0f, 0.0f, 0.0f, 0.0f, 0.0f, 0.0f, 0.0f, 0.0f,
                         0.0f, 0.0f, 0.0f, 0.0f, 0.0f, 0.0f, 0.0f, 0.0f, 0.0f};
      if (fam.usable) {
        if constexpr (PRETEST && WF) {
          if (pretest) {
            const bool miss3 = tile_misses_triangle<false, false, SlackProduct, true>(fam, {A1.z, A1.w, bz}, {A0.w, A1.x, A1.y}, {A0.x, A0.y, A0.z});
            asm volatile("" : "+v"(A0.x), "+v"(A0.y), "+v"(A0.z), "+v"(A0.w), "+v"(A1.x), "+v"(A1.y), "+v"(A1.z), "+v"(A1.w), "+v"(bz));
            keep = valid && !miss3 && !tile_misses_triangle<true>(fam, {A1.z, A1.w, bz}, {A0.w, A1.x, A1.y}, {A0.x, A0.y, A0.z}, forms);
          }
          else keep = valid && !tile_misses_triangle<false, false, SlackProduct, THIRD_WAVE>(fam, {A1.z, A1.w, bz}, {A0.w, A1.x, A1.y}, {A0.x, A0.y, A0.z});
        } else {
          keep = valid && !tile_misses_triangle<false, false, SlackProduct, THIRD_WAVE>(fam, {A1.z, A1.w, bz}, {A0.w, A1.x, A1.y}, {A0.x, A0.y, A0.z});
        }
      }
      const unsigned long long m = __builtin_amdgcn_ballot_w64(keep);
      if (count + static_cast<uint32_t>(__builtin_popcountll(m)) > L) break;
      const uint32_t pos = count + __builtin_amdgcn_mbcnt_hi(static_cast<uint32_t>(m >> 32),
                                                             __builtin_amdgcn_mbcnt_lo(static_cast<uint32_t>(m), 0u));
      if (keep) {
        cA[2u * pos] = A0;
        cA[2u * pos + 1u] = A1;
        cB[pos] = bz;
        cI[pos] = static_cast<int>(tri);
        if constexpr (PRETEST && WF) {
          if (pretest) {
            auto pk = [&](float hi, float lo) {
              const uint32_t h = __builtin_bit_cast(uint16_t, static_cast<_Float16>(hi)), l = __builtin_bit_cast(uint16_t, static_cast<_Float16>(lo));
              return __builtin_bit_cast(float, (h << 16) | l);
            };
            cP[4u * pos] = make_float4(forms[0], forms[1], forms[2], forms[3]);
            cP[4u * pos + 1u] = make_float4(forms[4], forms[5], forms[6], forms[7]);
            cP[4u * pos + 2u] = make_float4(forms[8], pk(forms[9], forms[10]), pk(forms[11], forms[12]), pk(forms[13], forms[14]));
            cP[4u * pos + 3u] = make_float4(pk(forms[15], forms[16]), pk(forms[17], 0.0f), 0.0f, 0.0f);
          }
        }
      }
      count += static_cast<uint32_t>(__builtin_popcountll(m));
      base += 64u;
    }
    __builtin_amdgcn_fence(__ATOMIC_RELEASE, "wavefront");
    __builtin_amdgcn_wave_barrier();
    list_count = count;
    if constexpr (STATS) { st_bin[0] += count; st_bin[1] += 1; }
    return base < src_count ? base : src_count;
  };

  if constexpr (Path == TracePath::SmallLists) {
    const size_t slot = (static_cast<size_t>(by) * gxb + bx) * 4u + wave;
    const uint32_t count = list_word & 0x3FFu;
    sure_hit_tile = loaded_sure;
    sure_winner = (list_word >> 10) & 0x3FFu;
    if (p.tile_lists != nullptr) {
      const uint32_t* const saved = p.tile_lists + slot * (1u + L);
      for (uint32_t base = 0; base < (sure_hit_tile ? 0u : count); base += 64u) {
        const uint32_t e = base + lane;
        if (e < count) {
          const uint32_t tri = saved[1u + e];
          cA[2u * e] = p.tri_a[2u * tri];
          cA[2u * e + 1u] = p.tri_a[2u * tri + 1u];
          cB[e] = p.tri_b[tri];
          cI[e] = static_cast<int>(tri);
        }
      }
    }
    __builtin_amdgcn_fence(__ATOMIC_RELEASE, "wavefront");
    __builtin_amdgcn_wave_barrier();
    list_count = count;
    if constexpr (STATS) { st_bin[0] += count; st_bin[1] += 1; }
    list_complete = true;
  }
  bool forms_ready = false;
  if constexpr (Path == TracePath::ClassifyForms) {
    const uint32_t next0 = classify(0u, std::true_type{});
    list_complete = next0 >= src_count;
    forms_ready = pretest && list_complete;
  }
  if constexpr (Path == TracePath::DenseLists) forms_ready = true;
  if constexpr (RNG_LATE) load_rng();
  tl_mark(1);
  float4 sure_col = make_float4(0.0f, 0.0f, 0.0f, 0.0f);
  const bool sure_sums = Path == TracePath::SmallLists && p.sure_table != nullptr;
  if constexpr (Path == TracePath::SmallLists) { if (sure_hit_tile) sure_col = sure_sums ? p.sure_table[sure_winner] : p.tri_color[sure_winner]; }
  if constexpr (STATS && Path == TracePath::SmallLists) {
    if (lane == 0u && p.stats != nullptr)
      atomicAdd(p.stats + (sure_hit_tile ? 13 : list_count == 0u ? 11 : list_count == 1u ? 12 : list_count == 2u ? 14 : 15), 1ull);
  }
  const uint32_t iters = FUSE ? p.iters : 1u;
  float rx = 0.0f, ry = 0.0f, rz = 0.0f, rw = 0.0f;
  for (uint32_t it = 0; it < iters; ++it) {
  if constexpr (FUSE) { ax = 0.0f; ay = 0.0f; az = 0.0f; }
  uint32_t traced_samples = p.samples;
  if constexpr (Path == TracePath::SmallLists) {
    if (sure_hit_tile) {
      rtd::rng_discard(rng, 3u * p.samples);
      if (sure_sums) { ax = sure_col.x; ay = sure_col.y; az = sure_col.z; }
      else for (uint32_t s = 0; s < p.samples; ++s) { ax += sure_col.x; ay += sure_col.y; az += sure_col.z; }
      if constexpr (STATS) st_pre += (p.samples + static_cast<uint32_t>(K) - 1u) / static_cast<uint32_t>(K);
      traced_samples = 0u;
    }
  }
  for (uint32_t s0 = 0; s0 < traced_samples; s0 += K) {
    if (s0 == static_cast<uint32_t>(K)) tl_mark(2);
    const uint32_t valid_k = (p.samples - s0 < static_cast<uint32_t>(K)) ? p.samples - s0 : static_cast<uint32_t>(K);
    V3 o[K], d[K];
    float best_t[K];
    int best_i[K];
#pragma unroll
    for (int k = 0; k < K; ++k) {
      if (static_cast<uint32_t>(k) < valid_k) get_ray<FMA>(p, focal, rng, o[k], d[k]);
      else { o[k] = {0.0f, 0.0f, 0.0f}; d[k] = {0.0f, 0.0f, -1.0f}; }
      best_t[k] = nearest ? FLT_MAX : -FLT_MAX;
      best_i[k] = -1;
    }

    const unsigned long long lanes_in = __builtin_amdgcn_ballot_w64(inside);
    unsigned long long pad_mask[K];
#pragma unroll
    for (int k = 0; k < K; ++k) pad_mask[k] = (static_cast<uint32_t>(k) < valid_k) ? 0ull : ~0ull;
    float dox[K], doy[K];
    float dFx = 0.0f, dFy = 0.0f, dFz = 0.0f;
    if constexpr (PRETEST) {
#pragma unroll
      for (int k = 0; k < K; ++k) { dox[k] = o[k].x - p.cam[9]; doy[k] = o[k].y - p.cam[10]; }
      dFx = focal.x - fam.fc[0]; dFy = focal.y - fam.fc[1]; dFz = focal.z - fam.fc[2];
    }
    if constexpr (Path == TracePath::SmallLists) {
      for (uint32_t j = 0; j < list_count; ++j) {
        const float4 A0 = cA[2u * j], A1 = cA[2u * j + 1u];
        test_triangle<FMA, K, FILTER, STATS>(A0, A1, [&] { return cB[j]; }, cI[j], o, d, best_t, best_i,
                                             nearest, inside, valid_k, st_exit, st_skip);
      }
    } else if constexpr (Path != TracePath::FullScan) {
      uint32_t base = 0;
      do {
        uint32_t next = src_count;
        if constexpr (Path != TracePath::DenseLists) {
          if (!list_complete) {
            next = classify(base, std::false_type{});
            if (base == 0u && next >= src_count) list_complete = true;
          }
        }
        auto forms_eval = [&](const float4 f0, const float4 f1, const float4 q2, const float4 q3) -> bool {
          const float f2 = q2.x;
          typedef _Float16 h2 __attribute__((ext_vector_type(2)));
          const h2 w0 = __builtin_bit_cast(h2, q2.y), w1 = __builtin_bit_cast(h2, q2.z), w2 = __builtin_bit_cast(h2, q2.w),
// ... 89 lines not shown
              const float4 n0 = p.tri_n[3 * win], n1 = p.tri_n[3 * win + 1], n2 = p.tri_n[3 * win + 2];
              const float w = (1.0f - u) - v;
              V3 m;
              if constexpr (FMA) {
                m.x = __builtin_fmaf(v, n2.x, __builtin_fmaf(u, n1.x, w * n0.x));
                m.y = __builtin_fmaf(v, n2.y, __builtin_fmaf(u, n1.y, w * n0.y));
                m.z = __builtin_fmaf(v, n2.z, __builtin_fmaf(u, n1.z, w * n0.z));
              } else {
                m.x = (w * n0.x + u * n1.x) + v * n2.x;
                m.y = (w * n0.y + u * n1.y) + v * n2.y;
                m.z = (w * n0.z + u * n1.z) + v * n2.z;
              }
              const V3 nn = M::normalize(m);
              r = rtd::absf(nn.x); g = rtd::absf(nn.y); b = rtd::absf(nn.z);
            } else if (by_slot) {
              r = cC[3 * win]; g = cC[3 * win + 1]; b = cC[3 * win + 2];
            } else {
              const float4 col = p.tri_color[win];
              r = col.x; g = col.y; b = col.z;
            }
          } else {
            const float4 sph = p.spheres[win - first_sphere];
            const V3 hp = {M::madd1(d[k].x, dist, o[k].x), M::madd1(d[k].y, dist, o[k].y),
                           M::madd1(d[k].z, dist, o[k].z)};
            const V3 nn = M::normalize(rtd::sub(hp, {sph.x, sph.y, sph.z}));
            r = rtd::absf(nn.x); g = rtd::absf(nn.y); b = rtd::absf(nn.z);
          }
        } else {
          if constexpr (FMA) {
            r = __builtin_fmaf(d[k].x, 0.2f, 0.15f * 0.8f);
            g = __builtin_fmaf(d[k].y, 0.2f, 0.11f * 0.8f);
            b = __builtin_fmaf(d[k].z, 0.2f, 0.13f * 0.8f);
          } else {
            r = 0.15f * 0.8f + d[k].x * 0.2f;
            g = 0.11f * 0.8f + d[k].y * 0.2f;
            b = 0.13f * 0.8f + d[k].z * 0.2f;
          }
        }
        ax += r; ay += g; az += b;
      }
    }
  }

  if constexpr (FUSE) {
    if (it == 0u && !(p.flags & TRACE_ZERO_ACC) && inside) {
      const float4 r0 = p.render[pix];
      rx = r0.x; ry = r0.y; rz = r0.z; rw = r0.w;
    }
    rx += ax; ry += ay; rz += az;
  }
  }
  tl_mark(3);
  uint32_t pix_lo = static_cast<uint32_t>(pix);
  asm volatile("" : "+v"(pix_lo));
  const size_t pix_e = pix_lo;
  if (inside) {
    float4 acc_in = make_float4(0.0f, 0.0f, 0.0f, 0.0f);
    if constexpr (!FUSE) {
      if (!(p.flags & TRACE_ZERO_ACC)) acc_in = p.render[pix_e];
    }
    const uint32_t cnt = p.count + iters * p.samples;
    float4 acc = acc_in;
    if constexpr (FUSE) {
      acc = make_float4(rx, ry, rz, rw);
    } else {
      acc.x += ax; acc.y += ay; acc.z += az;
    }
    p.render[pix_e] = acc;
    if (p.flags & TRACE_EMIT_IMAGE) {
      const float c = static_cast<float>(cnt);
      uint32_t bgra;
      if (!FUSE && sure_sums && sure_hit_tile && (p.flags & TRACE_ZERO_ACC)) bgra = __builtin_bit_cast(uint32_t, sure_col.w);
      else bgra = rtd::pack_color(255.0f * (acc.x / c), 255.0f * (acc.y / c), 255.0f * (acc.z / c));
      p.image[pix_e] = bgra;
      if (p.image_host != nullptr) p.image_host[pix_e] = bgra;
    }
    p.rng[1 * static_cast<size_t>(p.npix) + pix_e] = rng.v0;
    p.rng[2 * static_cast<size_t>(p.npix) + pix_e] = rng.v1;
    p.rng[3 * static_cast<size_t>(p.npix) + pix_e] = rng.v2;
    p.rng[4 * static_cast<size_t>(p.npix) + pix_e] = rng.v3;
    p.rng[5 * static_cast<size_t>(p.npix) + pix_e] = rng.v4;
  }
  tl_mark(4);
  if constexpr (STATS) {
    if (lane == 0 && p.stats != nullptr) {
#pragma unroll
      for (int e = 0; e < 4; ++e) {
        atomicAdd(p.stats + e, st_exit[e]);
        atomicAdd(p.stats + 4 + e, st_skip[e]);
      }
      atomicAdd(p.stats + 8, st_bin[0]);
      atomicAdd(p.stats + 9, st_bin[1]);
      atomicAdd(p.stats + 10, st_pre);
    }
  }
}


}
```

### raytracertest_amd/csrc/rt_tracer.hip

```cpp
#include "rt_tracer.hpp"

#include <map>

namespace rtr {

std::mutex g_err_mu;
std::string g_last_error;

void set_global_error(const std::string& s) {
  std::lock_guard<std::mutex> lk(g_err_mu);
  g_last_error = s;
  static const bool log = getenv("RT_MI355X_LOG") != nullptr;
  if (log) fprintf(stderr, "[rt_mi355x] %s\n", s.c_str());
}

std::mutex g_jump_mu;
std::vector<uint32_t> g_jump_host;
std::map<int, uint32_t*> g_jump_dev;

const std::vector<uint32_t>& jump_host() {
  std::lock_guard<std::mutex> lk(g_jump_mu);
  if (g_jump_host.empty()) g_jump_host = rth::build_jump_table();
  return g_jump_host;
}
// ... 158 lines not shown
  c.fov = Camera::radians(fov);
  c.focal = focalLength; c.aperture = aperture;
  c.transform();
  rc = guarded(t, [&] {
    t->use_device();
    t->stream = Stream(hipStreamNonBlocking);
    t->stream_b = Stream(hipStreamNonBlocking);
    int lo = 0, hi = 0;
    if (hipDeviceGetStreamPriorityRange(&lo, &hi) == hipSuccess && hi != lo) t->stream_l = Stream(hipStreamNonBlocking, hi);
    else t->stream_l = Stream(hipStreamNonBlocking);
    t->stagger_event = Event(hipEventDisableTiming);
    t->d_half_cost.ensure(2);
    HIP_CHECK(hipMemset(t->d_half_cost.get(), 0, 2 * sizeof(uint32_t)));
    HIP_CHECK(hipDeviceSynchronize());
    t->h_half_cost.ensure(1);
    *t->h_half_cost.get() = 0ull;
    t->lists.create(t->stream, t->stream_b, t->stream_l);
    t->handoff_event = Event(hipEventDisableTiming);
    t->join_event = Event(hipEventDisableTiming);
    t->fork_event = Event(hipEventDisableTiming);
    t->create_buffers();
  });
  if (rc != RT_OK) {
    std::string why = t->last_error;
    rt_tracer_destroy(t);
    set_global_error("rt_tracer_create: " + why);
    return rc;
  }
  *out = t;
  return RT_OK;
}

int rt_tracer_create(const uint32_t imageSize[2], const float cameraPosition[3],
                     const float cameraAngles[2], float fov, float focalLength, float aperture,
                     rt_tracer** out) {
  return rt_tracer_create_ex(imageSize, cameraPosition, cameraAngles, fov, focalLength, aperture,
                             nullptr, out);
}

void rt_tracer_destroy(rt_tracer* t) {
  if (!t) return;
  t->stopped = true;
  t->render.shutdown();
  if (t->mg) {
    multi_destroy(t);
    delete t;
    return;
  }
  member_leave(t);
  t->quiesce();
  delete t;
}

int rt_tracer_trace(rt_tracer* t, uint32_t iterationCount, uint32_t samplesPerIteration,
                    uint32_t updateInterval) {
  if (!t) return RT_ERR_INVALID;
  std::lock_guard<std::mutex> lk(t->api_mu);
  return guarded(t, [&] {
    t->cancel_and_join();
    t->completed = false;
    if (t->mg) t->render.run([=] { multi_trace_funct(t, iterationCount, samplesPerIteration, updateInterval); });
    else t->render.run([=] { t->trace_funct(iterationCount, samplesPerIteration, updateInterval); });
  });
}

void rt_tracer_stop(rt_tracer* t) {
  if (t) t->stopped = true;
}

int rt_tracer_wait(rt_tracer* t) {
  if (!t) return 0;
  std::lock_guard<std::mutex> lk(t->api_mu);
  t->render.wait_idle();
  t->stopped = false;
  return t->completed ? 1 : 0;
}

int rt_tracer_resize(rt_tracer* t, const uint32_t size[2]) {
  if (!t || !size || size[0] == 0 || size[1] == 0) return RT_ERR_INVALID;
  return exclusive(t, [&] {
    if (t->mg) { multi_resize(t, size[0], size[1]); return; }
    if (t->grp) throw HipFail{"Resize: the tracer is a member of a multi-process group (leave and re-join with the new bands)"};
    t->use_device();
    HIP_CHECK(hipStreamSynchronize(t->main_stream()));
    t->release_buffers();
    t->W = size[0];
    if (t->band_mode) {
      if (static_cast<uint64_t>(t->row0) + size[1] > t->H) throw HipFail{"row band exceeds full_height"};
      t->rows = size[1];
    } else {
      t->H = size[1]; t->rows = size[1];
    }
    t->create_buffers();
  });
}

void rt_tracer_set_camera_parameters(rt_tracer* t, float fov, float focalLength, float aperture) {
  if (!t) return;
  std::lock_guard<std::mutex> lk(t->state_mu);
  t->cam.fov = Camera::radians(fov);
  t->cam.focal = focalLength;
  t->cam.aperture = aperture;
}

void rt_tracer_rotate_camera(rt_tracer* t, const float angles[2]) {
  if (!t || !angles) return;
  std::lock_guard<std::mutex> lk(t->state_mu);
  t->cam.angles[0] += angles[0];
  t->cam.angles[1] += angles[1];
  t->cam.transform();
}

static int upload_scene_impl(rt_tracer* t, const rt_float4* hostData, size_t count, bool edges) {
  if (!t) return RT_ERR_INVALID;
  if (!hostData || count < 3 || count % 3 != 0) {
    t->set_error(fmt("UploadScene got invalid triangle list. Size = %zu", count));
    return RT_ERR_INVALID;
  }
  std::lock_guard<std::mutex> lk(t->api_mu);
  if (t->mg) {
    int rc = guarded(t, [&] { t->cancel_and_join(); multi_sync_all(t); });
    for (rt_tracer* b : t->mg->bands) {
      if (rc != RT_OK) break;
      rc = upload_scene_impl(b, hostData, count, edges);
      if (rc != RT_OK) t->set_error(b->last_error);
    }
    if (rc == RT_OK) { t->n_tris = static_cast<uint32_t>(count / 3); t->scene_generation++; }
    return rc;
  }
  return guarded(t, [&] {
    t->cancel_and_join();
    t->use_device();
    HIP_CHECK(hipStreamSynchronize(t->main_stream()));
    t->sync_list_stream();
    t->wait_queries();
    t->d_tri.reset(); t->d_tri_b.reset(); t->d_tri_color.reset(); t->d_tri_n.reset();
    t->n_tris = 0;
    const uint32_t n = static_cast<uint32_t>(count / 3);
    DevArray<float4> verts(count);
    t->d_tri.ensure(static_cast<size_t>(n) * 2); t->d_tri_b.ensure(n); t->d_tri_color.ensure(n);
    if (edges) t->d_tri_n.ensure(static_cast<size_t>(n) * 3);
    HIP_CHECK(hipMemcpyAsync(verts.get(), hostData, count * sizeof(float4), hipMemcpyHostToDevice, t->main_stream()));
    HIP_CHECK(rtk::launch_prep_triangles(t->fma, edges, verts.get(), n, t->d_tri.get(), t->d_tri_b.get(),
                                         t->d_tri_color.get(), t->d_tri_n.get(), t->main_stream()));
    HIP_CHECK(hipStreamSynchronize(t->main_stream()));
    t->n_tris = n;
    t->scene_generation++;
  });
}

int rt_tracer_upload_scene(rt_tracer* t, const rt_float4* hostData, size_t count) {
  return upload_scene_impl(t, hostData, count, false);
}

int rt_tracer_upload_scene_edges(rt_tracer* t, const rt_float4* hostData, size_t count) {
  return upload_scene_impl(t, hostData, count, true);
}

float rt_pack_normal(const float n[3]) {
  return floorf(n[0] * 127.0f + 127.5f) / 256.0f + floorf(n[1] * 127.0f + 127.5f) / 65536.0f +
         floorf(n[2] * 127.0f + 127.5f) / 16777216.0f;
}

void rt_unpack_normal(float packed, float n[3]) {
  const float m[3] = {1.0f, 256.0f, 65536.0f};
  for (int i = 0; i < 3; ++i) {
    const float s = packed * m[i];
    const float frac = s - floorf(s);
    n[i] = floorf(frac * 256.0f) / 127.0f - 1.0f;
  }
}

int rt_tracer_upload_spheres(rt_tracer* t, const rt_float4* spheres, size_t count) {
  if (!t || (count && !spheres)) return RT_ERR_INVALID;
  std::lock_guard<std::mutex> lk(t->api_mu);
  if (t->mg) {
    int rc = guarded(t, [&] { t->cancel_and_join(); multi_sync_all(t); });
    for (rt_tracer* b : t->mg->bands) {
      if (rc != RT_OK) break;
      rc = rt_tracer_upload_spheres(b, spheres, count);
      if (rc != RT_OK) t->set_error(b->last_error);
    }
    if (rc == RT_OK) t->n_spheres = static_cast<uint32_t>(count);
    return rc;
  }
  return guarded(t, [&] {
    t->cancel_and_join();
    t->use_device();
    HIP_CHECK(hipStreamSynchronize(t->main_stream()));
    t->wait_queries();
    t->d_spheres.reset();
    t->n_spheres = 0;
    if (count == 0) return;
    t->d_spheres.ensure(count);
    HIP_CHECK(hipMemcpy(t->d_spheres.get(), spheres, count * sizeof(float4), hipMemcpyHostToDevice));
    t->n_spheres = static_cast<uint32_t>(count);
  });
}

void rt_tracer_set_update_callback(rt_tracer* t, rt_callback_fn fn, void* user) {
  if (!t) return;
  std::lock_guard<std::mutex> lk(t->state_mu);
  t->update_cb = fn; t->update_user = user;
}

void rt_tracer_set_finished_callback(rt_tracer* t, rt_callback_fn fn, void* user) {
  if (!t) return;
  std::lock_guard<std::mutex> lk(t->state_mu);
  t->finished_cb = fn; t->finished_user = user;
}

int rt_tracer_set_seed(rt_tracer* t, uint64_t seed) {
  if (!t) return RT_ERR_INVALID;
  return exclusive(t, [&] {
    t->seed = seed;
    if (t->mg) {
      t->mg->opt.seed = seed;
      for (rt_tracer* b : t->mg->bands)
        if (rt_tracer_set_seed(b, seed) != RT_OK) throw HipFail{b->last_error};
      return;
    }
    t->use_device();
    t->create_states();
    HIP_CHECK(hipStreamSynchronize(t->main_stream()));
  });
}

static void trace_enqueue_once(rt_tracer* t, uint32_t iterationCount, uint32_t samplesPerIteration) {
  if (t->mg) { multi_trace_enqueue(t, iterationCount, samplesPerIteration); return; }
  if (t->grp) {
    const size_t k = member_band_index(t);
    const int b = t->grp->begin_frame();
    t->trace_enqueue_body(iterationCount, samplesPerIteration, t->grp->tile_target(k, b));
    t->grp->tile_written(k);
    t->grp->gather(b);
    return;
  }
  t->trace_enqueue_body(iterationCount, samplesPerIteration, t->image_mirror);
}

int rt_tracer_trace_enqueue(rt_tracer* t, uint32_t iterationCount, uint32_t samplesPerIteration) {
  return rt_tracer_trace_enqueue_n(t, iterationCount, samplesPerIteration, 1u);
}

int rt_tracer_trace_enqueue_n(rt_tracer* t, uint32_t iterationCount, uint32_t samplesPerIteration, uint32_t n_steps) {
  if (!t) return RT_ERR_INVALID;
  return exclusive(t, [&] {
    for (uint32_t s = 0; s < n_steps; ++s) trace_enqueue_once(t, iterationCount, samplesPerIteration);
  });
}

int rt_tracer_set_list_reuse(rt_tracer* t, int across_traces) {
  if (!t) return RT_ERR_INVALID;
  std::lock_guard<std::mutex> lk(t->api_mu);
  t->cancel_and_join();
  if (t->mg) for (rt_tracer* b : t->mg->bands) (void)rt_tracer_set_list_reuse(b, across_traces);
  t->reuse_across_traces = across_traces != 0;
  t->lists.key.reset();
  return RT_OK;
}

int rt_tracer_set_image_mirror(rt_tracer* t, void* device_visible_image) {
  if (!t) return RT_ERR_INVALID;
  std::lock_guard<std::mutex> lk(t->api_mu);
  if (t->mg || t->grp) { t->set_error("rt_tracer_set_image_mirror: the gather owns the second image target of a sharded frame"); return RT_ERR_STATE; }
  t->image_mirror = static_cast<uint32_t*>(device_visible_image);
  return RT_OK;
}

int rt_tracer_fused_iterations(rt_tracer* t, uint32_t samples) {
  if (t && t->mg) return static_cast<int>(t->mg->bands[0]->fused_iterations(samples));
  return t ? static_cast<int>(t->fused_iterations(samples)) : 0;
}

static void launch_impl(rt_tracer* t, uint32_t samples, uint32_t iterations, bool clear_first, bool emit) {
  if (t->mg) { multi_launch(t, samples, iterations, clear_first, emit); return; }
  t->use_device();
  const uint32_t flags = (clear_first ? rtk::TRACE_ZERO_ACC : 0u) | (emit ? rtk::TRACE_EMIT_IMAGE : 0u);
  if (t->grp && emit) {
    const size_t k = member_band_index(t);
    const int b = t->grp->begin_frame();
    t->enqueue_trace_launch(samples, flags, 0, iterations, t->grp->tile_target(k, b));
    t->grp->tile_written(k);
    t->grp->gather(b);
    return;
  }
  t->enqueue_trace_launch(samples, flags, 0, iterations, emit ? t->image_mirror : nullptr);
}

int rt_tracer_launch_iterations(rt_tracer* t, uint32_t samples, uint32_t iterations, int clear_first, int emit_image) {
  if (!t || iterations == 0u) return RT_ERR_INVALID;
  if (iterations > static_cast<uint32_t>(rt_tracer_fused_iterations(t, samples))) {
    t->set_error(fmt("rt_tracer_launch_iterations: %u iterations of %u samples exceed rt_tracer_fused_iterations", iterations, samples));
    return RT_ERR_INVALID;
  }
  return exclusive(t, [&] { launch_impl(t, samples, iterations, clear_first != 0, emit_image != 0); });
}

int rt_tracer_launch(rt_tracer* t, uint32_t samples, int clear_first, int emit_image) {
  return rt_tracer_launch_iterations(t, samples, 1u, clear_first, emit_image);
}

int rt_tracer_trace_stats(rt_tracer* t, uint32_t samples, uint64_t out[16]) {
  if (!t || !out) return RT_ERR_INVALID;
  std::lock_guard<std::mutex> lk(t->api_mu);
  if (t->mg) {
    memset(out, 0, 16 * sizeof(uint64_t));
    t->cancel_and_join();
    multi_push_camera(t);
    for (rt_tracer* b : t->mg->bands) {
      uint64_t part[16];
      const int rc = rt_tracer_trace_stats(b, samples, part);
      if (rc != RT_OK) { t->set_error(b->last_error); return rc; }
      for (int i = 0; i < 16; ++i) out[i] += part[i];
    }
    return RT_OK;
  }
  return guarded(t, [&] {
    t->cancel_and_join();
    t->use_device();
    DevArray<unsigned long long> counters(16);
    HIP_CHECK(hipMemsetAsync(counters.get(), 0, 16 * sizeof(unsigned long long), t->main_stream()));
    t->clear_accumulators();
    rtk::TraceParams p = t->params(samples);
    p.stats = counters.get();
    p.flags = t->mode_flags(p);
    t->launch_instrumented(p, samples);
    HIP_CHECK(hipMemcpy(out, counters.get(), 16 * sizeof(uint64_t), hipMemcpyDeviceToHost));
  });
}

int rt_tracer_sync(rt_tracer* t) {
  if (!t) return RT_ERR_INVALID;
  if (t->mg) return guarded(t, [&] { multi_sync_all(t); });
  return guarded(t, [&] {
    t->use_device();
    t->sync_all();
    if (t->grp) t->grp->sync();
  });
}

int rt_tracer_kernel_time(rt_tracer* t, double* total_ms, uint64_t* launches, int reset_after) {
  return read_clock(t, false, total_ms, launches, reset_after);
}
int rt_tracer_launch_time(rt_tracer* t, double* total_ms, uint64_t* launches, int reset_after) {
  return read_clock(t, true, total_ms, launches, reset_after);
}

size_t rt_tracer_buffer_bytes(rt_tracer* t, int which) { return t ? buffer_bytes(t, which) : 0; }
void* rt_tracer_device_pointer(rt_tracer* t, int which) {
  if (!t) return nullptr;
  if (!t->mg && (which == RT_BUF_RNG || which == RT_BUF_COUNTS) &&
      guarded(t, [&] { t->use_device(); t->materialise(which); }) != RT_OK) return nullptr;
  return buffer_ptr(t, which);
}

int rt_tracer_read_buffer(rt_tracer* t, int which, void* dst, size_t bytes) {
  if (!t || !dst) return RT_ERR_INVALID;
  if (t->mg) {
    if (bytes > buffer_bytes(t, which) || buffer_bytes(t, which) == 0) return RT_ERR_INVALID;
    return guarded(t, [&] { multi_read_buffer(t, which, dst, bytes); });
  }
  if (buffer_ptr(t, which) == nullptr || bytes > buffer_bytes(t, which)) return RT_ERR_INVALID;
  return guarded(t, [&] {
    t->use_device();
    t->materialise(which);
    HIP_CHECK(hipStreamSynchronize(t->main_stream()));
    if (t->grp) t->grp->sync();
    HIP_CHECK(hipMemcpy(dst, buffer_ptr(t, which), bytes, hipMemcpyDeviceToHost));
  });
}

int rt_tracer_copy_buffer_to_device(rt_tracer* t, int which, void* dst_device, size_t bytes) {
  if (!t || !dst_device || buffer_ptr(t, which) == nullptr || bytes > buffer_bytes(t, which)) return RT_ERR_INVALID;
  if (t->mg) return guarded(t, [&] {
    multi_sync_all(t);
    HIP_CHECK(hipSetDevice(t->mg->group.local[0].device));
    HIP_CHECK(hipMemcpy(dst_device, buffer_ptr(t, which), bytes, hipMemcpyDeviceToDevice));
  });
  return guarded(t, [&] {
    t->use_device();
    if (t->grp && which == RT_BUF_FRAME) t->grp->sync();
    t->materialise(which);
    HIP_CHECK(hipMemcpyAsync(dst_device, buffer_ptr(t, which), bytes, hipMemcpyDeviceToDevice, t->main_stream()));
    HIP_CHECK(hipStreamSynchronize(t->main_stream()));
  });
}

int rt_tracer_copy_buffer_to_device_async(rt_tracer* t, int which, void* dst_device, size_t bytes) {
  if (!t || !dst_device || buffer_ptr(t, which) == nullptr || bytes > buffer_bytes(t, which)) return RT_ERR_INVALID;
  if (t->mg || which == RT_BUF_FRAME) { t->set_error("rt_tracer_copy_buffer_to_device_async: per-stream copies are for plain tracers' own buffers"); return RT_ERR_STATE; }
  return guarded(t, [&] {
    t->use_device();
    t->materialise(which);
    HIP_CHECK(hipMemcpyAsync(dst_device, buffer_ptr(t, which), bytes, hipMemcpyDeviceToDevice, t->main_stream()));
  });
}

void* rt_tracer_stream(rt_tracer* t) { return (t && !t->mg) ? static_cast<void*>(t->stream) : nullptr; }
void* rt_tracer_stream_b(rt_tracer* t) { return (t && !t->mg) ? static_cast<void*>(t->stream_b) : nullptr; }

int rt_tracer_info(rt_tracer* t, uint32_t out[8]) {
  if (!t || !out) return RT_ERR_INVALID;
  if (t->mg) {
    (void)rt_tracer_info(t->mg->bands[0], out);
    out[3] = (t->W + 31) / 32; out[4] = (t->H + 7) / 8;
    out[7] = static_cast<uint32_t>(t->device);
    return RT_OK;
  }
  out[0] = t->last_k; out[1] = t->last_chunk; out[2] = t->last_lds;
  out[3] = (t->W + 31) / 32; out[4] = (t->rows + 7) / 8;
  out[5] = t->n_tris; out[6] = t->n_spheres; out[7] = static_cast<uint32_t>(t->device);
  return RT_OK;
}


int rt_tracer_create_multi(const uint32_t imageSize[2], const float cameraPosition[3], const float cameraAngles[2],
                           float fov, float focalLength, float aperture, const rt_options* options,
                           const int32_t* devices, uint32_t n_bands, rt_tracer** out) {
  return multi_create(imageSize, cameraPosition, cameraAngles, fov, focalLength, aperture, options, devices, n_bands, out);
}

int rt_group_unique_id(uint8_t id[RT_GROUP_ID_BYTES]) {
  if (!id) return RT_ERR_INVALID;
  return guarded(nullptr, [&] {
    ncclUniqueId uid;
    RCCL_CHECK(need_rccl().GetUniqueId(&uid));
    memcpy(id, uid.internal, RT_GROUP_ID_BYTES);
  });
}

static int join_impl(rt_tracer* t, uint32_t n_ranks, uint32_t rank, const uint8_t id[RT_GROUP_ID_BYTES], const uint32_t* row_begin) {
  if (!t || t->mg || n_ranks == 0u || rank >= n_ranks || (!id && n_ranks > 1u)) return RT_ERR_INVALID;
  static const uint8_t zero_id[RT_GROUP_ID_BYTES] = {0};
  return exclusive(t, [&] {
    member_join(t, n_ranks, rank, id ? id : zero_id, row_begin);
  });
}

int rt_tracer_join_group(rt_tracer* t, uint32_t n_ranks, uint32_t rank, const uint8_t id[RT_GROUP_ID_BYTES]) {
  return join_impl(t, n_ranks, rank, id, nullptr);
}

int rt_tracer_join_group_bands(rt_tracer* t, uint32_t n_ranks, uint32_t rank, const uint8_t id[RT_GROUP_ID_BYTES],
                               const uint32_t* row_begin) {
  return row_begin ? join_impl(t, n_ranks, rank, id, row_begin) : RT_ERR_INVALID;
}

int rt_balance_rows(uint32_t n_bands, const uint32_t* row_begin, const double* cost, uint32_t granule, uint32_t* new_row_begin) {
  if (n_bands == 0u || !row_begin || !cost || !new_row_begin) return RT_ERR_INVALID;
  for (uint32_t k = 0; k < n_bands; ++k) if (row_begin[k + 1] <= row_begin[k]) return RT_ERR_INVALID;
  balance_rows(n_bands, row_begin, cost, granule, new_row_begin);
  return RT_OK;
}

int rt_tracer_set_band(rt_tracer* t, uint32_t row_begin, uint32_t rows) {
  if (!t || t->mg || rows == 0u) return RT_ERR_INVALID;
  return exclusive(t, [&] {
    if (t->grp) throw HipFail{"rt_tracer_set_band: leave the group first"};
    if (!t->band_mode) throw HipFail{"rt_tracer_set_band: the tracer owns a whole image, not a band (rt_options.full_height)"};
    if (static_cast<uint64_t>(row_begin) + rows > t->H) throw HipFail{"row band exceeds full_height"};
    t->use_device();
    t->reshape(t->W, t->H, row_begin, rows);
  });
}

int rt_tracer_rebalance(rt_tracer* t) {
  if (!t || !t->mg) return RT_ERR_INVALID;
// ... 72 lines not shown
```

### raytracertest_amd/csrc/rt_tracer.hpp

```cpp
#pragma once
#include <algorithm>
#include <atomic>
#include <chrono>
#include <condition_variable>
#include <functional>
#include <cmath>
#include <cstdio>
#include <cstring>
#include <ctime>
#include <mutex>
#include <optional>
#include <string>
#include <thread>
#include <vector>

#include "../../include/rt_mi355x.h"
#include "rt_device_math.hpp"
#include "rt_hip_host.hpp"
#include "rt_kernels.hpp"
#include "rt_rng_host.hpp"

namespace rtr {

struct Env {
  bool log;
  bool no_split;
  bool no_pretest;
  bool no_sure_table;
  int row_interleave;
  long macro_cap;
  static bool on(const char* name) { const char* e = getenv(name); return e && e[0] == '1'; }
  Env() {
    log = getenv("RT_MI355X_LOG") != nullptr;
    no_split = on("RT_MI355X_NO_SPLIT");
    no_pretest = on("RT_MI355X_NO_PRETEST");
    no_sure_table = on("RT_MI355X_NO_SURE_TABLE");
    const char* ri = getenv("RT_MI355X_ROW_INTERLEAVE");
    row_interleave = (ri && (ri[0] == '0' || ri[0] == '1') && ri[1] == 0) ? ri[0] - '0' : -1;
    const char* mc = getenv("RT_MI355X_MACRO_CAP");
    macro_cap = mc ? strtol(mc, nullptr, 10) : 0;
  }
};

void set_global_error(const std::string& s);

const std::vector<uint32_t>& jump_host();
uint32_t* jump_device(int device);
constexpr size_t kJumpWords = 32u * 160u * 8u;

struct Camera {
  float position[3];
  float angles[2];
  float fov;
  float focal, aperture;
  float M[16];

  static float radians(float deg) { return deg * 0.01745329251994329576923690768489f; }

  void transform() {
    float sx, cx, sy, cy;
    rtd::sincos_spec(angles[0] * 0.5f, sx, cx);
    rtd::sincos_spec(angles[1] * 0.5f, sy, cy);
    const float Xw = cx, Xx = 1.0f * sx, Xy = 0.0f * sx, Xz = 0.0f * sx;
    const float Yw = cy, Yx = 0.0f * sy, Yy = 1.0f * sy, Yz = 0.0f * sy;
    const float w = Yw * Xw - Yx * Xx - Yy * Xy - Yz * Xz;
    const float x = Yw * Xx + Yx * Xw + Yy * Xz - Yz * Xy;
    const float y = Yw * Xy + Yy * Xw + Yz * Xx - Yx * Xz;
    const float z = Yw * Xz + Yz * Xw + Yx * Xy - Yy * Xx;
    const float qxx = x * x, qyy = y * y, qzz = z * z, qxz = x * z, qxy = x * y, qyz = y * z;
    const float qwx = w * x, qwy = w * y, qwz = w * z;
    memset(M, 0, sizeof M);
    M[0] = 1.0f - 2.0f * (qyy + qzz); M[1] = 2.0f * (qxy + qwz);        M[2] = 2.0f * (qxz - qwy);
    M[4] = 2.0f * (qxy - qwz);        M[5] = 1.0f - 2.0f * (qxx + qzz); M[6] = 2.0f * (qyz + qwx);
    M[8] = 2.0f * (qxz + qwy);        M[9] = 2.0f * (qyz - qwx);        M[10] = 1.0f - 2.0f * (qxx + qyy);
    M[15] = 1.0f;
  }
  float tan_half_fov() const {
    float s, c;
    rtd::sincos_spec(fov / 2.0f, s, c);
    return s / c;
  }
};

#ifndef RT_EVENT_STRIDE
#define RT_EVENT_STRIDE 16
#endif
#ifndef RT_PRETEST_LIST
#define RT_PRETEST_LIST 84u
#endif
struct EventPair { Event a, b, c; bool split = false; uint64_t seq = 0; };
class LaunchClock {
 public:
  static constexpr uint32_t kEventStride = RT_EVENT_STRIDE;
  bool start(bool waited, bool split, EventPair& e) {
    if (!waited && (counter_++ % kEventStride) != 0u) return false;
    std::lock_guard<std::mutex> lk(mu_);
    if (!free_.empty()) { e = std::move(free_.back()); free_.pop_back(); }
    else { e.a = Event::timing(); e.b = Event::timing(); e.c = Event::timing(); }
    e.split = split;
    return true;
  }
  void enqueued(EventPair e, int sync_after) {
    hipEvent_t wait_b = nullptr, wait_c = nullptr;
    size_t back = 2;
    {
      std::lock_guard<std::mutex> lk(mu_);
      if (sync_after == 0) reap_locked();
      e.seq = next_seq_++;
      pending_.push_back(std::move(e));
      back = (static_cast<size_t>(sync_after > 1 ? sync_after : 2) + kEventStride - 1u) / kEventStride;
      if (back < 2u) back = 2u;
      const EventPair* w = sync_after == 1 ? &pending_.back()
                           : (sync_after > 1 && pending_.size() >= back) ? &pending_[pending_.size() - back] : nullptr;
      if (w) { wait_b = w->b; wait_c = w->split ? w->c : nullptr; }
    }
    if (wait_b == nullptr) return;
    HIP_CHECK(hipEventSynchronize(wait_b));
    if (wait_c) HIP_CHECK(hipEventSynchronize(wait_c));
    if (sync_after > 1) drain(back - 1u);
  }
  void drain(size_t keep_last = 0) {
    std::lock_guard<std::mutex> lk(mu_);
    if (pending_.size() > keep_last) recycle_locked(pending_.size() - keep_last);
// ... 69 lines not shown
  void shutdown() {
    {
      std::unique_lock<std::mutex> lk(mu_);
      done_cv_.wait(lk, [&] { return !busy_.load(); });
      quit_ = true;
    }
    cv_.notify_one();
    if (th_.joinable()) th_.join();
  }

 private:
  static void spin_pause() {
#if defined(__x86_64__) || defined(__i386__)
    __builtin_ia32_pause();
#endif
  }
  void loop() {
    for (;;) {
      const auto t0 = std::chrono::steady_clock::now();
      while (!posted_.load(std::memory_order_acquire) &&
             std::chrono::steady_clock::now() - t0 < std::chrono::microseconds(50)) spin_pause();
      std::function<void()> job;
      {
        std::unique_lock<std::mutex> lk(mu_);
        cv_.wait(lk, [&] { return posted_.load() || quit_; });
        if (!posted_.load()) return;
        posted_.store(false);
        job = std::move(job_);
        job_ = nullptr;
      }
      job();
      {
        std::lock_guard<std::mutex> lk(mu_);
        busy_.store(false, std::memory_order_release);
      }
      done_cv_.notify_all();
    }
  }
  std::thread th_;
  std::mutex mu_;
  std::condition_variable cv_, done_cv_;
  std::function<void()> job_;
  std::atomic<bool> busy_{false}, posted_{false};
  bool quit_ = false;
};

struct ListKey {
  float cam[12], half_height, aspect, focal, aperture;
  uint32_t W, H, row0, rows, bin_list, n_tris, scene_generation;
  bool fma;
};
inline bool same_key(const std::optional<ListKey>& held, const ListKey& k) { return held && memcmp(&*held, &k, sizeof k) == 0; }

class TileListRing {
 public:
  static constexpr int kListRing = 8, kFreeEvents = 10;
  std::optional<ListKey> key;

  void create(hipStream_t a, hipStream_t b, hipStream_t l) {
    a_ = a; b_ = b; l_ = l;
    for (Event& e : list_ready_) e = Event(hipEventDisableTiming);
    for (int r = 0; r < kFreeEvents; ++r) { list_free_a_[r] = Event(hipEventDisableTiming); list_free_b_[r] = Event(hipEventDisableTiming); }
  }
  template <class Quiesce>
  bool prepare(size_t words, const ListKey& k, bool reuse, Quiesce&& quiesce) {
    if (words > words_) {
      quiesce();
      HIP_CHECK(hipStreamSynchronize(l_));
      release();
      const bool big = words * sizeof(uint32_t) > (size_t(128) << 20);
      ring_n_ = big ? 4 : 8; free_stride_ = big ? 2 : 4;
      for (int r = 0; r < ring_n_; ++r) {
        slots_[r].ensure(words);
        HIP_CHECK(hipMemsetAsync(slots_[r].get(), 0, words * sizeof(uint32_t), l_));
      }
      words_ = words;
    }
    if (reuse && same_key(key, k)) return false;
    key = k;
    return true;
  }
  uint64_t build_ahead() {
    const uint64_t m = builds_;
    if (m > 0 && m % free_stride_ == 0) {
      const int i = static_cast<int>((m / free_stride_) % kFreeEvents);
      HIP_CHECK(hipEventRecord(list_free_a_[i], a_));
      HIP_CHECK(hipEventRecord(list_free_b_[i], b_));
      free_build_[i] = m;
    }
    const int r = static_cast<int>(m % ring_n_);
    if (m >= alloc_build_ + ring_n_) {
      const uint64_t e = ((m - ring_n_ + 1 + free_stride_ - 1) / free_stride_) * free_stride_;
      const int i = static_cast<int>((e / free_stride_) % kFreeEvents);
      if (free_build_[i] != e) throw HipFail{"list ring: the free event of the slot's readers is missing"};
      if (e != free_waited_) {
        HIP_CHECK(hipStreamWaitEvent(l_, list_free_a_[i], 0));
        HIP_CHECK(hipStreamWaitEvent(l_, list_free_b_[i], 0));
        free_waited_ = e;
      }
    }
    cur_ = r;
    return m;
  }
  void built() { HIP_CHECK(hipEventRecord(list_ready_[cur_], l_)); ++builds_; }
  void wait(hipStream_t st, int which) {
    if (waited_[which] == builds_) return;
    HIP_CHECK(hipStreamWaitEvent(st, list_ready_[cur_], 0));
    waited_[which] = builds_;
  }
  void attach(rtk::TraceParams& p, uint32_t band_row0, bool have) const {
    const size_t slot_base = static_cast<size_t>((p.W + 31u) / 32u) * ((p.row0 - band_row0) / 8u) * 4u;
    p.tile_lists = have ? now() + slot_base * (1u + p.bin_list) : nullptr;
  }
  void release() {
    for (DevArray<uint32_t>& s : slots_) s.reset();
    words_ = 0; key.reset(); cur_ = 0; alloc_build_ = builds_;
  }
  uint32_t* now() const { return slots_[cur_].get(); }
  size_t words() const { return words_; }

 private:
  hipStream_t a_ = nullptr, b_ = nullptr, l_ = nullptr;
  int ring_n_ = 8, free_stride_ = 4;
  DevArray<uint32_t> slots_[kListRing];
  size_t words_ = 0;
  Event list_ready_[kListRing];
  Event list_free_a_[kFreeEvents], list_free_b_[kFreeEvents];
  uint64_t free_build_[kFreeEvents] = {};
  uint64_t alloc_build_ = 0;
  uint64_t free_waited_ = 0;
  int cur_ = 0;
  uint64_t builds_ = 0;
  uint64_t waited_[2] = {0, 0};
};

struct HalfLists {
  DevArray<uint32_t> macro, super, wave;
  std::optional<ListKey> macro_key;
  bool wave_valid = false;
  uint32_t wave_cap = 0;
  size_t wave_tiles = 0;
};

struct Group;
struct MultiState;

}

struct rt_tracer {
  rtr::Group* grp = nullptr;
  rtr::MultiState* mg = nullptr;
  rtr::Env env;
  int device = 0;
  uint32_t W = 0, H = 0;
  uint32_t row0 = 0, rows = 0;
  bool band_mode = false;
  uint64_t seed = 1;
  bool fma = true, filter = true, bin = true, nearest_hit = false;
  bool smooth_normals = false;
  uint32_t k_req = 0, chunk_req = 0, bin_list_req = 0;

  rtr::Stream stream;
  rtr::Stream stream_b;
  rtr::Stream stream_l;
  rtr::Stream stream_q;
  rtr::Event join_event, fork_event;
  bool b_dirty = false;
  bool a_dirty = false;
  bool split_launches = true;

  std::recursive_mutex order_mu;
  hipStream_t main_stream() {
    std::lock_guard<std::recursive_mutex> lk(order_mu);
    if (b_dirty) {
      HIP_CHECK(hipEventRecord(join_event, stream_b));
      HIP_CHECK(hipStreamWaitEvent(stream, join_event, 0));
      b_dirty = false;
    }
    a_dirty = true;
    return stream;
  }
  void fork_b() {
    std::lock_guard<std::recursive_mutex> lk(order_mu);
    if (!a_dirty) return;
    HIP_CHECK(hipEventRecord(fork_event, stream));
    HIP_CHECK(hipStreamWaitEvent(stream_b, fork_event, 0));
    a_dirty = false;
  }
  void mark_b_dirty() { std::lock_guard<std::recursive_mutex> lk(order_mu); b_dirty = true; }
  rtr::DevArray<float4> d_render;
  rtr::DevArray<uint32_t> d_counts, d_image, d_rng;
  uint32_t weyl_now = 0, count_now = 0;
  uint32_t weyl_plane = 0, count_plane = 0;
  bool weyl_plane_ok = false, count_plane_ok = false;
  void take_uniform_state(rtk::TraceParams& p) {
    if (p.flags & rtk::TRACE_ZERO_ACC) count_now = 0u;
    p.weyl = weyl_now; p.count = count_now;
    const uint32_t done = p.samples * (p.iters > 1u ? p.iters : 1u);
    weyl_now += 362437u * 3u * done;
    count_now += done;
  }
  void materialise(int which) {
    std::lock_guard<std::recursive_mutex> lk(order_mu);
    if (which == RT_BUF_RNG && !(weyl_plane_ok && weyl_plane == weyl_now) && d_rng.get() != nullptr) {
      HIP_CHECK(hipMemsetD32Async(reinterpret_cast<hipDeviceptr_t>(d_rng.get()), static_cast<int>(weyl_now), npix(), main_stream()));
      weyl_plane = weyl_now; weyl_plane_ok = true;
    }
    if (which == RT_BUF_COUNTS && !(count_plane_ok && count_plane == count_now) && d_counts.get() != nullptr) {
      HIP_CHECK(hipMemsetD32Async(reinterpret_cast<hipDeviceptr_t>(d_counts.get()), static_cast<int>(count_now), npix(), main_stream()));
      count_plane = count_now; count_plane_ok = true;
    }
  }
  rtr::PinnedArray<uint32_t> h_image;
  rtr::PinnedArray<uint32_t> h_image_alt;
// ... 6 lines not shown
  rtr::DevArray<float4> d_tri_n;
  uint32_t n_tris = 0;
  rtr::DevArray<float4> d_spheres;
  uint32_t n_spheres = 0;
  rtr::DevArray<float> d_q_rays;
  rtr::DevArray<uint32_t> d_q_pixels;
  rtr::DevArray<float4> d_q_hits;
  rtr::DevArray<float> d_q_segs;
  rtr::DevArray<uint8_t> d_q_occluded;
  rtr::Event query_done;
  void wait_queries() { if (query_done) HIP_CHECK(hipEventSynchronize(query_done)); }
  uint32_t query_accel = RT_QUERY_SCAN;
  uint32_t query_slack_milli = 1000u;
  rtr::DevArray<float4> d_bvh_nodes, d_bvh_records;
  bool bvh_built = false;
  uint32_t bvh_scene = 0;
  uint64_t bvh_info[6] = {0, 0, 0, 0, 0, 0};
  uint32_t bvh_leaf_records = 0;
  bool bvh_valid() const { return bvh_built && bvh_scene == scene_generation; }

  std::mutex state_mu;
  rtr::Camera cam;
  rt_callback_fn update_cb = nullptr; void* update_user = nullptr;
  rt_callback_fn finished_cb = nullptr; void* finished_user = nullptr;

  std::mutex api_mu;
  rtr::RenderThread render;
  std::atomic<bool> stopped{false};
  std::atomic<bool> completed{false};

  rtr::LaunchClock clock;

  std::mutex err_mu;
  std::string last_error;
  uint32_t last_k = 0, last_chunk = 0, last_lds = 0;

  void set_error(const std::string& s) {
    { std::lock_guard<std::mutex> lk(err_mu); last_error = s; }
    rtr::set_global_error(s);
  }
  uint32_t npix() const { return W * rows; }
  void use_device() { HIP_CHECK(hipSetDevice(device)); }

  void cancel_and_join() {
    if (render.busy()) {
      stopped = true;
      render.wait_idle();
      stopped = false;
    }
  }

  void release_buffers() {
    d_render.reset(); d_counts.reset(); d_image.reset(); d_rng.reset(); h_image.reset(); h_image_alt.reset();
  }

  void quiesce() {
    (void)hipSetDevice(device);
    for (const rtr::Stream* s : {&stream_b, &stream, &stream_l, &stream_q}) if (*s) (void)hipStreamSynchronize(*s);
    if (query_done) (void)hipEventSynchronize(query_done);
    clock.drain();
  }

  void create_states() {
    uint32_t seeded[6];
    rth::seed_state(seed, seeded);
    const uint32_t p0 = row0 * W;
    if (static_cast<uint64_t>(W) * H > 0xFFFFFFFFull) throw rtr::HipFail{"frames above 2^32 pixels are not supported (32-bit pixel index, Kernels.cuh:128)"};
    uint32_t* const tables = rtr::jump_device(device);
    std::lock_guard<std::recursive_mutex> lk(order_mu);
    HIP_CHECK(rtk::launch_rng_init(d_rng.get(), npix(), p0, seeded, tables, tables + rtr::kJumpWords, main_stream()));
    weyl_now = seeded[0]; weyl_plane_ok = false;
  }

  void create_buffers() {
    const size_t n = npix();
    if (n == 0) throw rtr::HipFail{"image has no pixels"};
    d_rng.ensure(n * 6); d_render.ensure(n); d_counts.ensure(n); d_image.ensure(n); h_image.ensure(n); h_image_alt.ensure(n);
    memset(h_image.get(), 0, n * sizeof(uint32_t));
    memset(h_image_alt.get(), 0, n * sizeof(uint32_t));
    HIP_CHECK(hipMemsetAsync(d_render.get(), 0, n * sizeof(float4), main_stream()));
    HIP_CHECK(hipMemsetAsync(d_image.get(), 0, n * sizeof(uint32_t), main_stream()));
    { std::lock_guard<std::recursive_mutex> lk(order_mu); count_now = 0u; count_plane_ok = false; }
    create_states();
    HIP_CHECK(hipStreamSynchronize(main_stream()));
  }

  void reshape(uint32_t w, uint32_t h, uint32_t r0, uint32_t n) {
    HIP_CHECK(hipStreamSynchronize(main_stream()));
    sync_list_stream();
    release_buffers();
    W = w; H = h; row0 = r0; rows = n;
    lists.key.reset();
    create_buffers();
  }

  void copy_image_to(uint32_t* target) {
    HIP_CHECK(hipMemcpyAsync(target, d_image.get(), static_cast<size_t>(npix()) * sizeof(uint32_t), hipMemcpyDeviceToDevice, main_stream()));
  }

  void tile_corner_bound(rtk::TraceParams& p) const {
    p.tile_curv = -1.0f; p.tile_round = 0.0f;
    double G[3][3];
    for (int i = 0; i < 3; ++i)
      for (int j = 0; j < 3; ++j) {
        G[i][j] = 0.0;
        for (int r = 0; r < 3; ++r) G[i][j] += static_cast<double>(p.cam[i * 3 + r]) * static_cast<double>(p.cam[j * 3 + r]);
      }
    double lmax = 0.0, lmin = 1e300;
    for (int i = 0; i < 3; ++i) {
      const double off = std::fabs(G[i][(i + 1) % 3]) + std::fabs(G[i][(i + 2) % 3]);
      lmax = std::max(lmax, G[i][i] + off);
      lmin = std::min(lmin, G[i][i] - off);
    }
    if (!(lmin > 0.25) || !(lmax < 4.0)) return;
    const double hh = std::fabs(static_cast<double>(p.half_height)), asp = std::fabs(static_cast<double>(p.aspect));
    const double a = 7.0 * 2.0 * hh * asp / static_cast<double>(W), b = 7.0 * 2.0 * hh / static_cast<double>(H);
    if (!(0.5 * (a * a + b * b) * (lmax / lmin) <= 0.1 * std::min(a, b))) return;
    const double foc = std::fabs(static_cast<double>(p.focal));
#ifndef RT_TILE_CURV_SCALE
#define RT_TILE_CURV_SCALE 1.0
#endif
    const double curv = foc * 0.5 * (a * a + b * b) * (lmax / lmin) * 1.001 * RT_TILE_CURV_SCALE + 1e-30;
    const double pos = std::max(std::fabs(p.cam[9]), std::max(std::fabs(p.cam[10]), std::fabs(p.cam[11])));
    const double round = foc * (1.0 + hh * asp + hh) + pos;
    if (!(curv <= 1e30) || !(round <= 1e30)) return;
    p.tile_curv = std::nextafter(static_cast<float>(curv), 3.0e38f);
    p.tile_round = std::nextafter(static_cast<float>(round), 3.0e38f);
  }

  rtk::TraceParams params(uint32_t samples) {
    rtk::TraceParams p;
    memset(&p, 0, sizeof p);
    rtr::Camera c;
    { std::lock_guard<std::mutex> lk(state_mu); c = cam; }
    p.render = d_render.get(); p.rng = d_rng.get();
    p.W = W; p.H = H; p.row0 = row0; p.rows = rows; p.npix = npix(); p.samples = samples;
    for (int col = 0; col < 4; ++col)
      for (int r = 0; r < 3; ++r) p.cam[col * 3 + r] = c.M[col * 4 + r];
    p.half_height = c.tan_half_fov();
    p.aspect = static_cast<float>(W) / static_cast<float>(H);
    p.focal = c.focal; p.aperture = c.aperture;
    tile_corner_bound(p);
    p.tri_a = d_tri.get(); p.tri_b = d_tri_b.get(); p.tri_color = d_tri_color.get(); p.n_tris = n_tris;
    p.tri_n = smooth_normals ? d_tri_n.get() : nullptr;
    p.stats = nullptr;
    p.spheres = d_spheres.get(); p.n_spheres = n_spheres;
    p.chunk = chunk_req ? chunk_req : 1024u;
    if (p.chunk > 4096u) p.chunk = 4096u;
    uint32_t want = bin_list_req ? bin_list_req : ((n_tris + 31u) / 32u) * 32u;
    want = ((want + 31u) / 32u) * 32u;
    p.bin_list = want < 32u ? 32u : want > (bin_list_req ? 960u : 256u) ? (bin_list_req ? 960u : 256u) : want;
    p.block_list = n_tris > p.bin_list ? 1024u : 0u;
    if (p.block_list != 0u && !bin_list_req) p.bin_list = 192u;
    if (pretest && filter && bin && n_tris >= kPretestMinTris && n_tris <= 50000u) {
      p.pretest_on = 1u;
      if (!bin_list_req) p.bin_list = RT_PRETEST_LIST;
      else p.bin_list = (p.bin_list + 1u) & ~1u;
      if (p.block_list != 0u) p.block_list = 448u;
    }
    return p;
  }

  uint32_t mode_flags(const rtk::TraceParams& p) const {
    return (nearest_hit ? rtk::TRACE_NEAREST_HIT : 0u) | (p.pretest_on ? rtk::TRACE_PRETEST : 0u) |
           (sure_hit ? 0u : rtk::TRACE_NO_SURE_HIT);
  }

  int pick_k(uint32_t samples) const {
    if (k_req == 1 || k_req == 2 || k_req == 4) return static_cast<int>(k_req);
    const uint32_t want = (n_tris <= 128u) ? 2u : 4u;
    return samples >= want ? static_cast<int>(want) : samples >= 2 ? 2 : 1;
  }

  void enqueue_trace_launch(uint32_t samples, uint32_t flags, int sync_after, uint32_t iters = 1,
                            uint32_t* host_image = nullptr, bool allow_split = true) {
    const int K = pick_k(samples);
    rtk::TraceParams p = params(samples);
    p.iters = iters;
    p.image_host = host_image;
    p.flags = flags | mode_flags(p);
    p.image = d_image.get();
    const rtk::TracePath path = trace_path(p);
    bool have_lists = false;
    const bool build_lists = prepare_tile_lists(p, path, (flags & rtk::TRACE_ZERO_ACC) != 0u, have_lists);
    attach_sure_table(p, have_lists);
    last_k = K; last_chunk = p.chunk;
    last_lds = rtk::trace_lds_bytes(p, path == rtk::TracePath::DenseLists ? rtk::TracePath::ClassifyForms : path);
    const uint32_t r0 = allow_split ? split_row(p.rows) : 0u;
    rtr::EventPair e;
    const bool timed = clock.start(sync_after == 1, r0 != 0u, e);
    std::unique_lock<std::recursive_mutex> uniform_lk(order_mu);
    take_uniform_state(p);
    if (r0 == 0u) {
      (void)main_stream();
      if (build_lists) build_tile_lists_ahead(p);
      lists.attach(p, row0, have_lists);
      if (timed) HIP_CHECK(hipEventRecord(e.a, stream));
      if (have_lists) lists.wait(stream, 0);
      attach_macro_lists(p, path, 0, stream, (flags & rtk::TRACE_ZERO_ACC) != 0u);
      HIP_CHECK(rtk::launch_trace(p, fma, filter, path, K, stream));
      if (timed) HIP_CHECK(hipEventRecord(e.b, stream));
    } else {
      fork_b();
      if (build_lists) build_tile_lists_ahead(p);
      const bool stagger = stagger_next.exchange(false);
      const bool interleave = have_lists && want_interleave();
      if (have_lists && interleave != rows_interleaved) {
        (void)main_stream();
        fork_b();
        rows_interleaved = interleave;
        if (env.log) fprintf(stderr, "[rt_mi355x] split launches: halves by %s\n", interleave ? "even / odd block rows" : "rows");
      }
      rtk::TraceParams half[2] = {sub_band(p, 0u, r0), sub_band(p, r0, p.rows - r0)};
      if (interleave) { half[0] = p; half[1] = p; half[0].row_il = half[1].row_il = 1u; half[1].row_phase = 1u; }
      hipStream_t st[2] = {stream, stream_b};
      if (timed) HIP_CHECK(hipEventRecord(e.a, stream));
      for (int h = 0; h < 2; ++h) {
        lists.attach(half[h], row0, have_lists);
        if (have_lists) lists.wait(st[h], h);
        if (h == 1 && stagger) {
          const uint32_t us = static_cast<uint32_t>(clock.last_half_ms() * 450.0f);
          if (us >= 5u) HIP_CHECK(rtk::launch_delay(us, stream_b));
          else HIP_CHECK(hipStreamWaitEvent(stream_b, stagger_event, 0));
        }
        const rtk::TracePath half_path = trace_path(half[h]);
        attach_macro_lists(half[h], half_path, h, st[h], (flags & rtk::TRACE_ZERO_ACC) != 0u);
        HIP_CHECK(rtk::launch_trace(half[h], fma, filter, half_path, K, st[h]));
        if (h == 0 && stagger) HIP_CHECK(hipEventRecord(stagger_event, stream));
      }
      if (timed) { HIP_CHECK(hipEventRecord(e.b, stream)); HIP_CHECK(hipEventRecord(e.c, stream_b)); }
      mark_b_dirty();
    }
    uniform_lk.unlock();
    if (timed) clock.enqueued(std::move(e), sync_after);
  }

  static rtk::TraceParams sub_band(const rtk::TraceParams& p, uint32_t off, uint32_t n) {
    rtk::TraceParams q = p;
    const size_t px = static_cast<size_t>(off) * p.W;
    q.row0 = p.row0 + off; q.rows = n;
    q.render = p.render + px; q.rng = p.rng + px;
    q.image = p.image + px;
    if (p.image_host != nullptr) q.image_host = p.image_host + px;
    return q;
  }

  void clear_accumulators() {
    std::lock_guard<std::recursive_mutex> lk(order_mu);
    HIP_CHECK(hipMemsetAsync(d_render.get(), 0, static_cast<size_t>(npix()) * sizeof(float4), main_stream()));
    count_now = 0u;
  }

  void convert() {
    std::lock_guard<std::recursive_mutex> lk(order_mu);
    HIP_CHECK(rtk::launch_convert(d_render.get(), count_now, d_image.get(), npix(), main_stream()));
  }

  static void sync_polling(hipStream_t st) {
    const auto t0 = std::chrono::steady_clock::now();
    for (;;) {
      const hipError_t e = hipStreamQuery(st);
      if (e == hipSuccess) return;
      if (e != hipErrorNotReady) HIP_CHECK(e);
      if (std::chrono::steady_clock::now() - t0 > std::chrono::milliseconds(2)) break;
    }
    (void)hipGetLastError();
    HIP_CHECK(hipStreamSynchronize(st));
  }

  void fetch_image() {
    HIP_CHECK(hipMemcpyAsync(h_image.get(), d_image.get(), static_cast<size_t>(npix()) * sizeof(uint32_t),
                             hipMemcpyDeviceToHost, main_stream()));
    HIP_CHECK(hipStreamSynchronize(main_stream()));
  }

  rtr::TileListRing lists;
  rtr::Event stagger_event;
  std::atomic<bool> stagger_next{true};
  rtr::DevArray<uint32_t> d_half_cost;
  rtr::PinnedArray<unsigned long long> h_half_cost;
  bool rows_interleaved = false;
  bool want_interleave() {
    if (env.row_interleave >= 0) return env.row_interleave != 0;
    if (h_half_cost.get() == nullptr) return false;
    const unsigned long long w = *reinterpret_cast<volatile unsigned long long*>(h_half_cost.get());
    const double u = static_cast<double>(w & 0xFFFFFFFFull), l = static_cast<double>(w >> 32);
    if (u + l < 16.0) return rows_interleaved;
    const double ratio = (u > l ? u : l) / ((u > l ? l : u) + 1.0);
    return rows_interleaved ? ratio > 1.15 : ratio > 1.25;
  }
  uint32_t split_row(uint32_t band_rows) const {
    return (split_launches && band_rows >= 128u) ? ((band_rows / 2u + 7u) / 8u) * 8u : 0u;
  }
  void sync_list_stream() { if (stream_l) HIP_CHECK(hipStreamSynchronize(stream_l)); }
  void sync_all() {
    const uint64_t seen = clock.seq_now();
    HIP_CHECK(hipStreamSynchronize(main_stream()));
    sync_list_stream();
    stagger_next = true;
    clock.drain_before(seen);
  }
  uint32_t scene_generation = 0;

  rtr::ListKey make_key(const rtk::TraceParams& p, uint32_t bin_word) const {
    rtr::ListKey k;
    memset(&k, 0, sizeof k);
    memcpy(k.cam, p.cam, sizeof k.cam);
    k.half_height = p.half_height; k.aspect = p.aspect; k.focal = p.focal; k.aperture = p.aperture;
    k.W = p.W; k.H = p.H; k.row0 = p.row0; k.rows = p.rows; k.bin_list = bin_word; k.n_tris = p.n_tris;
    k.scene_generation = scene_generation; k.fma = fma;
    return k;
  }

  bool prepare_tile_lists(const rtk::TraceParams& p, rtk::TracePath path, bool first_launch_of_trace, bool& have) {
    have = path == rtk::TracePath::SmallLists && p.n_tris != 0u;
    if (!have) return false;
    const size_t tiles = static_cast<size_t>((W + 31u) / 32u) * ((rows + 7u) / 8u + 1u) * 4u;
    return lists.prepare(tiles * (1u + p.bin_list), make_key(p, p.bin_list), !(first_launch_of_trace && !reuse_across_traces),
                         [&] { HIP_CHECK(hipStreamSynchronize(main_stream())); });
  }

  rtr::DevArray<float4> d_sure_table;
  uint32_t sure_table_samples = 0;
  uint64_t sure_table_scene = ~0ull;
  void attach_sure_table(rtk::TraceParams& p, bool have) {
    p.sure_table = nullptr;
    if (!have || env.no_sure_table || p.n_tris == 0u) return;
    if (sure_table_samples != p.samples || sure_table_scene != scene_generation || d_sure_table.size() < p.n_tris) {
      hipStream_t st = main_stream();
      if (d_sure_table.size() < p.n_tris) {
        HIP_CHECK(hipStreamSynchronize(st));
        d_sure_table.ensure(p.n_tris);
      }
      HIP_CHECK(rtk::launch_sure_table(p.tri_color, p.n_tris, p.samples, d_sure_table.get(), st));
      sure_table_samples = p.samples; sure_table_scene = scene_generation;
    }
    p.sure_table = d_sure_table.get();
  }

  void build_tile_lists_ahead(const rtk::TraceParams& p_band) {
    const uint64_t m = lists.build_ahead();
    rtk::TraceParams q = p_band;
    lists.attach(q, row0, true);
    const uint32_t sr = split_row(rows);
    if (sr != 0u && d_half_cost.get() != nullptr && env.row_interleave < 0 && (m % 32u) == 0u) { q.half_cost = d_half_cost.get(); q.cost_split_brow = sr / 8u; }
    HIP_CHECK(rtk::launch_tile_lists(q, fma, stream_l));
    lists.built();
    if (q.half_cost != nullptr) HIP_CHECK(rtk::launch_publish_half_cost(d_half_cost.get(), h_half_cost.get(), stream_l));
  }

  void launch_instrumented(rtk::TraceParams& p, uint32_t samples) {
    const rtk::TracePath path = trace_path(p);
    bool have_lists = false;
    (void)prepare_tile_lists(p, path, true, have_lists);
    sync_list_stream();
    lists.attach(p, row0, have_lists);
    if (have_lists) HIP_CHECK(rtk::launch_tile_lists(p, fma, main_stream()));
    attach_macro_lists(p, path, 0, main_stream());
    {
      std::lock_guard<std::recursive_mutex> lk(order_mu);
      take_uniform_state(p);
      HIP_CHECK(rtk::launch_trace(p, fma, filter, path, pick_k(samples), main_stream()));
    }
    HIP_CHECK(hipStreamSynchronize(main_stream()));
  }

  rtr::HalfLists half_lists[2];
  bool macro = true;
  bool pretest = true;
  bool sure_hit = true;
  bool reuse_across_traces = true;
  static constexpr uint32_t kPretestMinTris = 4096;
  static constexpr uint32_t kMacroW = 128, kMacroH = 64, kMacroCapMax = 65536;
#ifndef RT_SUPER_F
#define RT_SUPER_F 4
#endif
  static constexpr uint32_t kSuperF = RT_SUPER_F, kSuperMinTris = 2048;
  bool super_level = true;

  void attach_macro_lists(rtk::TraceParams& p, rtk::TracePath path, int half, hipStream_t st, bool first_launch_of_trace = true) {
    p.macro_lists = nullptr;
    if (!macro || path == rtk::TracePath::FullScan || path == rtk::TracePath::SmallLists) return;
    rtr::HalfLists& h = half_lists[half];
    p.macro_w = kMacroW; p.macro_h = kMacroH;
    p.macro_nx = (p.W + p.macro_w - 1u) / p.macro_w;
    const uint32_t ny = (p.rows + p.macro_h - 1u) / p.macro_h;
    p.macro_cap = p.n_tris < kMacroCapMax ? p.n_tris : kMacroCapMax;
    if (env.macro_cap > 0 && static_cast<uint32_t>(env.macro_cap) < p.macro_cap) p.macro_cap = static_cast<uint32_t>(env.macro_cap);
    if (h.macro.ensure(static_cast<size_t>(p.macro_nx) * ny * (p.macro_cap + 1u))) h.macro_key.reset();
    p.macro_lists = h.macro.get();
    p.super_lists = nullptr; p.macro_bounds = nullptr; p.super_f = 0u; p.super_chunks = 0u; p.super_nx = 0u;
    const uint32_t chunks = (p.n_tris + rtk::kSuperChunk - 1u) / rtk::kSuperChunk;
    if (super_level && p.n_tris >= kSuperMinTris && chunks <= rtk::kSuperMaxChunks && p.macro_nx * ny > kSuperF * kSuperF) {
      p.super_f = kSuperF; p.super_chunks = chunks;
      p.super_nx = (p.macro_nx + kSuperF - 1u) / kSuperF;
      const size_t sw = static_cast<size_t>(p.super_nx) * ((ny + kSuperF - 1u) / kSuperF) * chunks * (rtk::kSuperChunk + 1u) +
                        static_cast<size_t>(p.macro_nx) * ny * 8u;
      if (h.super.ensure(sw)) h.macro_key.reset();
      p.super_lists = h.super.get();
      p.macro_bounds = reinterpret_cast<float*>(h.super.get() + (sw - static_cast<size_t>(p.macro_nx) * ny * 8u));
    }
    const rtr::ListKey k = make_key(p, p.macro_cap * 65536u + p.macro_w * 256u + p.macro_h);
    const bool same = rtr::same_key(h.macro_key, k) && !(first_launch_of_trace && !reuse_across_traces);
    if (!same) {
      h.macro_key = k;
      if (p.super_lists != nullptr) HIP_CHECK(rtk::launch_super_bin(p, fma, st));
      HIP_CHECK(rtk::launch_macro_bin(p, fma, st));
    }
    attach_wave_lists(p, path, h, st, !same);
  }

  static constexpr size_t kWaveListsMaxBytes = size_t(6) << 30;
  static size_t wave_list_tiles(const rtk::TraceParams& p) { return static_cast<size_t>((p.W + 31u) / 32u) * ((p.rows + 7u) / 8u) * 4u; }
  static size_t wave_list_words(const rtk::TraceParams& p) { return wave_list_tiles(p) * (1u + p.bin_list) * 16u; }
  void attach_wave_lists(rtk::TraceParams& p, rtk::TracePath path, rtr::HalfLists& h, hipStream_t st, bool macro_rebuilt) {
    p.wave_lists = nullptr; p.wave_cap = 0u;
    if (macro_rebuilt) h.wave_valid = false;
    if (path != rtk::TracePath::DenseLists) return;
    if (h.wave.ensure(wave_list_words(p))) h.wave_valid = false;
    p.wave_lists = h.wave.get(); p.wave_cap = p.bin_list;
    if (!h.wave_valid) {
      HIP_CHECK(rtk::launch_wave_lists(p, fma, st));
      h.wave_valid = true; h.wave_cap = p.bin_list; h.wave_tiles = wave_list_tiles(p);
    }
  }

  rtk::TracePath trace_path(const rtk::TraceParams& p) const {
    if (!bin) return rtk::TracePath::FullScan;
    if (p.n_tris <= p.bin_list) return rtk::TracePath::SmallLists;
    if (!p.pretest_on || !filter) return rtk::TracePath::Classify;
    if (p.stats != nullptr || !macro || wave_list_words(p) * sizeof(uint32_t) > kWaveListsMaxBytes) return rtk::TracePath::ClassifyForms;
    return rtk::TracePath::DenseLists;
  }

  static constexpr int kWindow = 4;

  void trace_enqueue_body(uint32_t iterationCount, uint32_t samplesPerIteration, uint32_t* target) {
    use_device();
    if (iterationCount == 0) {
      clear_accumulators();
      convert();
      if (target) copy_image_to(target);
      return;
    }
    const uint32_t group = fused_iterations(samplesPerIteration);
    for (uint32_t i = 0; i < iterationCount;) {
      const uint32_t n = iterationCount - i < group ? iterationCount - i : group;
      const bool last = i + n == iterationCount;
      enqueue_trace_launch(samplesPerIteration, (i == 0 ? rtk::TRACE_ZERO_ACC : 0u) | (last ? rtk::TRACE_EMIT_IMAGE : 0u),
                           0, n, last ? target : nullptr);
      i += n;
    }
  }

  uint32_t fused_iterations(uint32_t samplesPerIteration) {
    if (samplesPerIteration == 0u || !rtk::trace_can_fuse(trace_path(params(samplesPerIteration)), filter)) return 1u;
    const uint32_t n = 64u / samplesPerIteration;
    return n < 1u ? 1u : n;
  }

  void trace_funct(uint32_t iterationCount, uint32_t samplesPerIteration, uint32_t updateInterval) {
    try {
      use_device();
      bool cleared = false;
      struct { bool due = false; uint32_t* image = nullptr; rt_callback_fn cb = nullptr; void* user = nullptr; } pend;
      auto deliver = [&] {
        if (!pend.due) return;
        HIP_CHECK(hipEventSynchronize(handoff_event));
        pend.cb(pend.image, static_cast<size_t>(npix()) * sizeof(uint32_t), pend.user);
        pend.due = false;
      };
      uint32_t* final_image = h_image.get();
      uint32_t i = 0;
      while (!stopped && i < iterationCount) {
        rt_callback_fn cb; void* user;
        { std::lock_guard<std::mutex> lk(state_mu); cb = update_cb; user = update_user; }
        auto is_update = [&](uint32_t k) { return cb != nullptr && k > 0 && updateInterval > 0 && k % updateInterval == 0; };
        const uint32_t last_allowed = iterationCount - 1u - i < fused_iterations(samplesPerIteration) - 1u
                                          ? iterationCount - 1u : i + fused_iterations(samplesPerIteration) - 1u;
        uint32_t e = i;
        while (e < last_allowed && !is_update(e)) ++e;
        const bool update = is_update(e);
        const bool emit = update || e + 1 == iterationCount;
        const uint32_t flags = (cleared ? 0u : rtk::TRACE_ZERO_ACC) | (emit ? rtk::TRACE_EMIT_IMAGE : 0u);
        uint32_t* const target = emit ? (handoff_next ? h_image_alt : h_image).get() : nullptr;
        if (emit && pend.due && pend.image == target) deliver();
        enqueue_trace_launch(samplesPerIteration, flags, kWindow, e - i + 1u, target, false);
        cleared = true;
        deliver();
        if (emit) { final_image = target; handoff_next ^= 1; }
        if (update) {
          HIP_CHECK(hipEventRecord(handoff_event, main_stream()));
          pend.due = true; pend.image = target; pend.cb = cb; pend.user = user;
        }
        i = e + 1u;
      }
      deliver();
      clock.drain();
      if (!cleared) {
        clear_accumulators();
        if (!stopped) convert();
      }
      if (stopped) { HIP_CHECK(hipStreamSynchronize(main_stream())); return; }
      if (cleared && i == iterationCount) {
        sync_polling(main_stream());
      } else {
        fetch_image();
        final_image = h_image.get();
      }
      completed = true;
      rt_callback_fn cb; void* user;
      { std::lock_guard<std::mutex> lk(state_mu); cb = finished_cb; user = finished_user; }
      if (cb != nullptr) cb(final_image, static_cast<size_t>(npix()) * sizeof(uint32_t), user);
    } catch (const rtr::HipFail& f) {
      set_error(f.what);
    } catch (...) {
      set_error("unknown failure in the render thread");
    }
  }
};

#include "rt_multi.hpp"

namespace rtr {

template <class F>
int guarded(rt_tracer* t, F&& f) {
  auto fail = [t](const std::string& why, int rc) { if (t) t->set_error(why); else set_global_error(why); return rc; };
  try {
    f();
    return RT_OK;
  } catch (const HipFail& e) {
    return fail(e.what, RT_ERR_HIP);
  } catch (const std::exception& e) {
    return fail(e.what(), RT_ERR_STATE);
  } catch (...) {
    return fail("unknown failure", RT_ERR_STATE);
  }
}

template <class F>
int exclusive(rt_tracer* t, F&& f) {
  std::lock_guard<std::mutex> lk(t->api_mu);
  return guarded(t, [&] { t->cancel_and_join(); f(); });
}

int require_device(int device);
void multi_push_camera(rt_tracer* t);

}
```

Before: 598,600.

## Tag tile lists with build generation to drop the cross-stream wait

Each tile-list word now carries a generation tag in its upper bits. The trace kernel compares that tag with the expected one and, if the list is stale or partly foreign, falls back to scanning every triangle. Because of this, the trace launch no longer waits on the list-build stream's event unless the tracer is resuming from idle, so list building and tracing can overlap. The cost is extra tag checks and a retry ballot in the kernel, a slot memset when tags wrap, and slower full scans whenever a tile reads a list that is not yet written.

```diff
diff --git a/include/rt_mi355x.h b/include/rt_mi355x.h
--- a/include/rt_mi355x.h
+++ b/include/rt_mi355x.h
@@ -150,6 +150,9 @@
 int rt_dbg_check_midrange(int device, uint64_t out[4]);
 int rt_dbg_wave_list_counts(rt_tracer* t, int half, uint32_t* dst, size_t capacity_tiles, uint32_t* n_tiles, uint32_t* capacity_per_tile);
 int rt_dbg_read_tile_lists(rt_tracer* t, uint32_t* dst, size_t capacity_words, uint32_t* words_per_tile);
+int rt_dbg_set_list_tag_skew(rt_tracer* t, uint32_t skew);
+int rt_dbg_list_fallbacks(rt_tracer* t, int enable, uint64_t* count, int reset);
+int rt_dbg_clear_list_tags(rt_tracer* t, const uint64_t* word_indices, size_t n);
 int rt_dbg_focal_boxes(rt_tracer* t, float curv_scale, float* boxes, size_t boxes_capacity, float* focal, size_t focal_capacity);
 int rt_dbg_classify(rt_tracer* t, uint32_t level, uint32_t forms, uint32_t slack_milli, const uint32_t* regions, uint32_t n_regions,
                     float* out, size_t capacity_floats);
diff --git a/raytracertest_amd/api.py b/raytracertest_amd/api.py
--- a/raytracertest_amd/api.py
+++ b/raytracertest_amd/api.py
@@ -35,7 +35,7 @@
     "rt_dbg_rng_init_host",
     "rt_tracer_create_multi", "rt_group_unique_id", "rt_tracer_join_group", "rt_tracer_leave_group",
     "rt_tracer_gather_time", "rt_tracer_band_count", "rt_tracer_band_info",
-    "rt_tracer_join_group_bands", "rt_balance_rows", "rt_tracer_rebalance", "rt_tracer_set_band", "rt_dbg_read_tile_lists", "rt_dbg_wave_list_counts", "rt_dbg_focal_boxes", "rt_dbg_classify",
+    "rt_tracer_join_group_bands", "rt_balance_rows", "rt_tracer_rebalance", "rt_tracer_set_band", "rt_dbg_read_tile_lists", "rt_dbg_set_list_tag_skew", "rt_dbg_list_fallbacks", "rt_dbg_clear_list_tags", "rt_dbg_wave_list_counts", "rt_dbg_focal_boxes", "rt_dbg_classify",
     "rt_tracer_gather_only", "rt_tracer_group_info",
     "rt_tracer_intersect", "rt_tracer_intersect_device", "rt_tracer_pick", "rt_tracer_focus_at",
     "rt_tracer_occluded", "rt_tracer_occluded_device",
@@ -197,6 +197,9 @@
         L.rt_tracer_set_band.argtypes = [vp, C.c_uint32, C.c_uint32]
         L.rt_dbg_read_tile_lists.argtypes = [vp, u32p, C.c_size_t, u32p]
         L.rt_dbg_wave_list_counts.argtypes = [vp, C.c_int, u32p, C.c_size_t, u32p, u32p]
+        L.rt_dbg_set_list_tag_skew.argtypes = [vp, C.c_uint32]
+        L.rt_dbg_list_fallbacks.argtypes = [vp, C.c_int, C.POINTER(C.c_uint64), C.c_int]
+        L.rt_dbg_clear_list_tags.argtypes = [vp, C.POINTER(C.c_uint64), C.c_size_t]
         L.rt_dbg_focal_boxes.argtypes = [vp, C.c_float, f32p, C.c_size_t, f32p, C.c_size_t]
         L.rt_tracer_gather_only.argtypes = [vp]
         L.rt_tracer_group_info.argtypes = [vp, C.c_char_p, C.c_size_t]
@@ -480,6 +483,18 @@
         self._check(self._lib.rt_dbg_wave_list_counts(self._h, half, _u32p(buf), buf.size, _u32p(n), _u32p(cap)))
         return buf[:int(n[0])].copy(), int(cap[0])
 
+    def DebugSetListTagSkew(self, skew):
+        self._check(self._lib.rt_dbg_set_list_tag_skew(self._h, int(skew)))
+
+    def DebugListFallbacks(self, enable=True, reset=False):
+        n = C.c_uint64(0)
+        self._check(self._lib.rt_dbg_list_fallbacks(self._h, 1 if enable else 0, C.byref(n), 1 if reset else 0))
+        return int(n.value)
+
+    def DebugClearListTags(self, word_indices):
+        idx = np.ascontiguousarray(word_indices, np.uint64)
+        self._check(self._lib.rt_dbg_clear_list_tags(self._h, idx.ctypes.data_as(C.POINTER(C.c_uint64)), idx.size))
+
     def DebugTileListWords(self):
         bx, by = (self.width + 31) // 32, (self.rows + 7) // 8
         wpt = np.zeros(1, np.uint32)
diff --git a/raytracertest_amd/csrc/rt_debug.hip b/raytracertest_amd/csrc/rt_debug.hip
--- a/raytracertest_amd/csrc/rt_debug.hip
+++ b/raytracertest_amd/csrc/rt_debug.hip
@@ -91,7 +91,49 @@
     if (!t->lists.now() || !t->lists.key) throw HipFail{"no tile lists (small scenes build them ahead of their first trace launch)"};
     const size_t n = t->lists.words() < capacity_words ? t->lists.words() : capacity_words;
     HIP_CHECK(hipMemcpy(dst, t->lists.now(), n * sizeof(uint32_t), hipMemcpyDeviceToHost));
+    for (size_t i = 0; i < n; ++i) dst[i] &= ~rtk::kListTagMask;
     if (words_per_tile) *words_per_tile = 1u + t->lists.key->bin_list;
+  });
+}
+
+int rt_dbg_set_list_tag_skew(rt_tracer* t, uint32_t skew) {
+  if (!t || t->mg || skew > rtk::kListTags) return RT_ERR_INVALID;
+  return on_tracer(t, [&] { t->lists.tag_skew = skew; });
+}
+
+int rt_dbg_list_fallbacks(rt_tracer* t, int enable, uint64_t* count, int reset) {
+  if (!t || t->mg) return RT_ERR_INVALID;
+  return on_tracer(t, [&] {
+    t->sync_main();
+    if (t->d_list_fallbacks.get() == nullptr) {
+      t->d_list_fallbacks.ensure(1);
+      HIP_CHECK(hipMemset(t->d_list_fallbacks.get(), 0, sizeof(unsigned long long)));
+    }
+    if (count) {
+      unsigned long long v = 0;
+      HIP_CHECK(hipMemcpy(&v, t->d_list_fallbacks.get(), sizeof v, hipMemcpyDeviceToHost));
+      *count = v;
+    }
+    if (reset) HIP_CHECK(hipMemset(t->d_list_fallbacks.get(), 0, sizeof(unsigned long long)));
+    HIP_CHECK(hipDeviceSynchronize());
+    t->lists.fallbacks = enable ? t->d_list_fallbacks.get() : nullptr;
+  });
+}
+
+int rt_dbg_clear_list_tags(rt_tracer* t, const uint64_t* word_indices, size_t n) {
+  if (!t || t->mg || (!word_indices && n != 0)) return RT_ERR_INVALID;
+  return on_tracer(t, [&] {
+    t->sync_main();
+    t->sync_list_stream();
+    if (!t->lists.now() || !t->lists.key) throw HipFail{"no tile lists (small scenes build them ahead of their first trace launch)"};
+    std::vector<uint32_t> w(t->lists.words());
+    HIP_CHECK(hipMemcpy(w.data(), t->lists.now(), w.size() * sizeof(uint32_t), hipMemcpyDeviceToHost));
+    for (size_t i = 0; i < n; ++i) {
+      if (word_indices[i] >= w.size()) throw HipFail{fmt("word %llu is outside the lists (%zu words)", static_cast<unsigned long long>(word_indices[i]), w.size())};
+      w[word_indices[i]] &= ~rtk::kListTagMask;
+    }
+    HIP_CHECK(hipMemcpy(t->lists.now(), w.data(), w.size() * sizeof(uint32_t), hipMemcpyHostToDevice));
+    HIP_CHECK(hipDeviceSynchronize());
   });
 }
 
diff --git a/raytracertest_amd/csrc/rt_kernels.hpp b/raytracertest_amd/csrc/rt_kernels.hpp
--- a/raytracertest_amd/csrc/rt_kernels.hpp
+++ b/raytracertest_amd/csrc/rt_kernels.hpp
@@ -48,7 +48,10 @@
   uint32_t* wave_lists;
   uint32_t  wave_cap;
   uint32_t  flags;
+  unsigned long long* list_fallbacks;
+  uint32_t  list_tag;
 };
+constexpr uint32_t kListTagShift = 20u, kListTags = 2047u, kListTagMask = kListTags << kListTagShift;
 
 constexpr uint32_t TRACE_ZERO_ACC = 1u;
 constexpr uint32_t TRACE_EMIT_IMAGE = 2u;
diff --git a/raytracertest_amd/csrc/rt_lists.hpp b/raytracertest_amd/csrc/rt_lists.hpp
--- a/raytracertest_amd/csrc/rt_lists.hpp
+++ b/raytracertest_amd/csrc/rt_lists.hpp
@@ -256,6 +256,7 @@
   const TileFamily fam = make_family<SL>(p, b);
 
   uint32_t* const saved = p.tile_lists + static_cast<size_t>(sl) * (1u + p.bin_list);
+  const uint32_t tagw = p.list_tag << kListTagShift;
   const uint32_t n = p.n_tris;
   uint32_t count = 0;
   const float NEG = -__builtin_inff();
@@ -279,7 +280,7 @@
     const unsigned long long m = __builtin_amdgcn_ballot_w64(keep);
     const unsigned long long gm = G == 64 ? m : ((m >> gbase) & 0xFFFFFFFFull);
     const uint32_t pos = count + static_cast<uint32_t>(__builtin_popcountll(gm & ((1ull << gl) - 1ull)));
-    if (keep) saved[1u + pos] = tri;
+    if (keep) saved[1u + pos] = tri | tagw;
     count += static_cast<uint32_t>(__builtin_popcountll(gm));
     const bool cand = keep && sure && fam.usable;
     const float Qs = group_max<G>(cand ? q[0] : NEG);
@@ -308,7 +309,7 @@
     const float R = (I1 == A) ? M2 : M1;
     sure_one = count <= 1u || (R < Q - 1e-4f * (__builtin_fabsf(R) + __builtin_fabsf(Q)));
   }
-  if (live && gl == 0u) saved[0] = count | (A << 10) | (sure_one ? 0x80000000u : 0u);
+  if (live && gl == 0u) saved[0] = count | (A << 10) | (sure_one ? 0x80000000u : 0u) | tagw;
 }
 
 template <class SL>
@@ -380,6 +381,7 @@
   const bool tile_valid = mine.any;
   const TileFamily fam = make_family<SL>(p, mine);
   uint32_t* const saved = p.tile_lists + static_cast<size_t>(tile_valid ? tslot : 0u) * (1u + p.bin_list);
+  const uint32_t tagw = p.list_tag << kListTagShift;
   const float NEG = -__builtin_inff();
   uint32_t count = 0;
   bool haveA = false;
@@ -402,7 +404,7 @@
     }
     const uint32_t gm = static_cast<uint32_t>(__builtin_amdgcn_ballot_w64(keep) >> gsh) & GM;
     const uint32_t pos = count + static_cast<uint32_t>(__builtin_popcount(gm & ((1u << j) - 1u)));
-    if (keep) saved[1u + pos] = tri;
+    if (keep) saved[1u + pos] = tri | tagw;
     count += static_cast<uint32_t>(__builtin_popcount(gm));
     const bool cd = keep && sure && fam.usable;
     const float Qs = max_group<G2>(cd ? q[0] : NEG);
@@ -438,10 +440,8 @@
     sure_one = count <= 1u || (R < Q - 1e-4f * (__builtin_fabsf(R) + __builtin_fabsf(Q)));
     if (one_pass) sure_one = sure_one || others_ok;
   }
-  if (j == 0u) {
-    if (tile_valid) saved[0] = count | (A << 10) | (sure_one ? 0x80000000u : 0u);
-    else if (slot_live) p.tile_lists[static_cast<size_t>(tslot) * (1u + p.bin_list)] = 0u;
-  }
+  if (j == 0u && (tile_valid || slot_live))
+    p.tile_lists[static_cast<size_t>(tslot) * (1u + p.bin_list)] = count | (A << 10) | (sure_one ? 0x80000000u : 0u) | tagw;
   if (p.half_cost != nullptr) {
     const bool rays = j == 0u && tile_valid && !sure_one;
     const uint32_t nu = static_cast<uint32_t>(__builtin_popcountll(__builtin_amdgcn_ballot_w64(rays && !lower)));
diff --git a/raytracertest_amd/csrc/rt_trace.hpp b/raytracertest_amd/csrc/rt_trace.hpp
--- a/raytracertest_amd/csrc/rt_trace.hpp
+++ b/raytracertest_amd/csrc/rt_trace.hpp
@@ -147,13 +147,14 @@
 
 
   const bool sure_ok = Path == TracePath::SmallLists && (p.flags & (TRACE_NEAREST_HIT | TRACE_NO_SURE_HIT)) == 0u && p.n_spheres == 0u && p.tri_n == nullptr;
-  bool loaded_sure = false;
+  bool loaded_sure = false, list_stale = false;
   uint32_t list_word = 0u;
   if constexpr (Path == TracePath::SmallLists) {
     if (p.tile_lists != nullptr) {
       const size_t slot0 = (static_cast<size_t>(by) * gxb + bx) * 4u + wave;
       list_word = static_cast<uint32_t>(__builtin_amdgcn_readfirstlane(static_cast<int>(p.tile_lists[slot0 * (1u + p.bin_list)])));
-      loaded_sure = sure_ok && (list_word >> 31) != 0u;
+      list_stale = ((list_word >> kListTagShift) & kListTags) != p.list_tag;
+      loaded_sure = sure_ok && !list_stale && (list_word >> 31) != 0u;
     }
   }
   V3 po = {0.0f, 0.0f, 0.0f}, pd = {0.0f, 0.0f, 0.0f}, focal = {0.0f, 0.0f, 0.0f};
@@ -345,20 +346,32 @@
 
   if constexpr (Path == TracePath::SmallLists) {
     const size_t slot = (static_cast<size_t>(by) * gxb + bx) * 4u + wave;
-    const uint32_t count = list_word & 0x3FFu;
+    uint32_t count = list_word & 0x3FFu;
     sure_hit_tile = loaded_sure;
     sure_winner = (list_word >> 10) & 0x3FFu;
     if (p.tile_lists != nullptr) {
       const uint32_t* const saved = p.tile_lists + slot * (1u + L);
-      for (uint32_t base = 0; base < (sure_hit_tile ? 0u : count); base += 64u) {
-        const uint32_t e = base + lane;
-        if (e < count) {
-          const uint32_t tri = saved[1u + e];
-          cA[2u * e] = p.tri_a[2u * tri];
-          cA[2u * e + 1u] = p.tri_a[2u * tri + 1u];
-          cB[e] = p.tri_b[tri];
-          cI[e] = static_cast<int>(tri);
-        }
+      if (list_stale) count = n;
+      for (;;) {
+        bool foreign = false;
+        for (uint32_t base = 0; base < (sure_hit_tile ? 0u : count); base += 64u) {
+          const uint32_t e = base + lane;
+          if (e < count) {
+            uint32_t tri = e;
+            if (!list_stale) {
+              const uint32_t w = saved[1u + e];
+              const bool mine = (w >> kListTagShift) == p.list_tag;
+              foreign = foreign || !mine;
+              tri = mine ? (w & 0x3FFu) : 0u;
+            }
+            cA[2u * e] = p.tri_a[2u * tri];
+            cA[2u * e + 1u] = p.tri_a[2u * tri + 1u];
+            cB[e] = p.tri_b[tri];
+            cI[e] = static_cast<int>(tri);
+          }
+        }
+        if (list_stale || __builtin_amdgcn_ballot_w64(foreign) == 0ull) break;
+        list_stale = true; count = n;
       }
     }
     __builtin_amdgcn_fence(__ATOMIC_RELEASE, "wavefront");
@@ -614,6 +627,10 @@
     p.rng[5 * static_cast<size_t>(p.npix) + pix_e] = rng.v4;
   }
   tl_mark(4);
+  if constexpr (Path == TracePath::SmallLists) {
+    if (list_stale && p.list_fallbacks != nullptr && __builtin_amdgcn_mbcnt_hi(~0u, __builtin_amdgcn_mbcnt_lo(~0u, 0u)) == 0u)
+      atomicAdd(p.list_fallbacks, 1ull);
+  }
   if constexpr (STATS) {
     if (lane == 0 && p.stats != nullptr) {
 #pragma unroll
diff --git a/raytracertest_amd/csrc/rt_tracer.hip b/raytracertest_amd/csrc/rt_tracer.hip
--- a/raytracertest_amd/csrc/rt_tracer.hip
+++ b/raytracertest_amd/csrc/rt_tracer.hip
@@ -264,7 +264,7 @@
     if (t->mg) { multi_resize(t, size[0], size[1]); return; }
     if (t->grp) throw HipFail{"Resize: the tracer is a member of a multi-process group (leave and re-join with the new bands)"};
     t->use_device();
-    HIP_CHECK(hipStreamSynchronize(t->main_stream()));
+    t->sync_main();
     t->release_buffers();
     t->W = size[0];
     if (t->band_mode) {
@@ -313,7 +313,7 @@
   return guarded(t, [&] {
     t->cancel_and_join();
     t->use_device();
-    HIP_CHECK(hipStreamSynchronize(t->main_stream()));
+    t->sync_main();
     t->sync_list_stream();
     t->wait_queries();
     t->d_tri.reset(); t->d_tri_b.reset(); t->d_tri_color.reset(); t->d_tri_n.reset();
@@ -325,7 +325,7 @@
     HIP_CHECK(hipMemcpyAsync(verts.get(), hostData, count * sizeof(float4), hipMemcpyHostToDevice, t->main_stream()));
     HIP_CHECK(rtk::launch_prep_triangles(t->fma, edges, verts.get(), n, t->d_tri.get(), t->d_tri_b.get(),
                                          t->d_tri_color.get(), t->d_tri_n.get(), t->main_stream()));
-    HIP_CHECK(hipStreamSynchronize(t->main_stream()));
+    t->sync_main();
     t->n_tris = n;
     t->scene_generation++;
   });
@@ -369,7 +369,7 @@
   return guarded(t, [&] {
     t->cancel_and_join();
     t->use_device();
-    HIP_CHECK(hipStreamSynchronize(t->main_stream()));
+    t->sync_main();
     t->wait_queries();
     t->d_spheres.reset();
     t->n_spheres = 0;
@@ -404,7 +404,7 @@
     }
     t->use_device();
     t->create_states();
-    HIP_CHECK(hipStreamSynchronize(t->main_stream()));
+    t->sync_main();
   });
 }
 
@@ -439,6 +439,7 @@
   if (t->mg) for (rt_tracer* b : t->mg->bands) (void)rt_tracer_set_list_reuse(b, across_traces);
   t->reuse_across_traces = across_traces != 0;
   t->lists.key.reset();
+  t->lists_idle = true;
   return RT_OK;
 }
 
@@ -547,7 +548,7 @@
   return guarded(t, [&] {
     t->use_device();
     t->materialise(which);
-    HIP_CHECK(hipStreamSynchronize(t->main_stream()));
+    t->sync_main();
     if (t->grp) t->grp->sync();
     HIP_CHECK(hipMemcpy(dst, buffer_ptr(t, which), bytes, hipMemcpyDeviceToHost));
   });
@@ -565,7 +566,7 @@
     if (t->grp && which == RT_BUF_FRAME) t->grp->sync();
     t->materialise(which);
     HIP_CHECK(hipMemcpyAsync(dst_device, buffer_ptr(t, which), bytes, hipMemcpyDeviceToDevice, t->main_stream()));
-    HIP_CHECK(hipStreamSynchronize(t->main_stream()));
+    t->sync_main();
   });
 }
 
diff --git a/raytracertest_amd/csrc/rt_tracer.hpp b/raytracertest_amd/csrc/rt_tracer.hpp
--- a/raytracertest_amd/csrc/rt_tracer.hpp
+++ b/raytracertest_amd/csrc/rt_tracer.hpp
@@ -29,6 +29,7 @@
   bool no_sure_table;
   int row_interleave;
   long macro_cap;
+  int list_wait;
   static bool on(const char* name) { const char* e = getenv(name); return e && e[0] == '1'; }
   Env() {
     log = getenv("RT_MI355X_LOG") != nullptr;
@@ -39,6 +40,8 @@
     row_interleave = (ri && (ri[0] == '0' || ri[0] == '1') && ri[1] == 0) ? ri[0] - '0' : -1;
     const char* mc = getenv("RT_MI355X_MACRO_CAP");
     macro_cap = mc ? strtol(mc, nullptr, 10) : 0;
+    const char* lw = getenv("RT_MI355X_LIST_WAIT");
+    list_wait = (lw && (lw[0] == '0' || lw[0] == '1') && lw[1] == 0) ? lw[0] - '0' : -1;
   }
 };
 
@@ -274,6 +277,7 @@
   }
   uint64_t build_ahead() {
     const uint64_t m = builds_;
+    tag_ = 1u + static_cast<uint32_t>(m % rtk::kListTags);
     if (m > 0 && m % free_stride_ == 0) {
       const int i = static_cast<int>((m / free_stride_) % kFreeEvents);
       HIP_CHECK(hipEventRecord(list_free_a_[i], a_));
@@ -290,6 +294,7 @@
         HIP_CHECK(hipStreamWaitEvent(l_, list_free_b_[i], 0));
         free_waited_ = e;
       }
+      if (m % rtk::kListTags < static_cast<uint64_t>(ring_n_)) HIP_CHECK(hipMemsetAsync(slots_[r].get(), 0, words_ * sizeof(uint32_t), l_));
     }
     cur_ = r;
     return m;
@@ -303,10 +308,16 @@
   void attach(rtk::TraceParams& p, uint32_t band_row0, bool have) const {
     const size_t slot_base = static_cast<size_t>((p.W + 31u) / 32u) * ((p.row0 - band_row0) / 8u) * 4u;
     p.tile_lists = have ? now() + slot_base * (1u + p.bin_list) : nullptr;
-  }
+    p.list_tag = tag_ ^ tag_skew;
+    p.list_fallbacks = have ? fallbacks : nullptr;
+  }
+  uint32_t tag() const { return tag_; }
+  uint32_t tag_in_stream() { if (tag_ == 0u) tag_ = rtk::kListTags; return tag_; }
+  uint32_t tag_skew = 0;
+  unsigned long long* fallbacks = nullptr;
   void release() {
     for (DevArray<uint32_t>& s : slots_) s.reset();
-    words_ = 0; key.reset(); cur_ = 0; alloc_build_ = builds_;
+    words_ = 0; key.reset(); cur_ = 0; alloc_build_ = builds_; tag_ = 0;
   }
   uint32_t* now() const { return slots_[cur_].get(); }
   size_t words() const { return words_; }
@@ -322,6 +333,7 @@
   uint64_t alloc_build_ = 0;
   uint64_t free_waited_ = 0;
   int cur_ = 0;
+  uint32_t tag_ = 0;
   uint64_t builds_ = 0;
   uint64_t waited_[2] = {0, 0};
 };
@@ -494,11 +506,11 @@
     HIP_CHECK(hipMemsetAsync(d_image.get(), 0, n * sizeof(uint32_t), main_stream()));
     { std::lock_guard<std::recursive_mutex> lk(order_mu); count_now = 0u; count_plane_ok = false; }
     create_states();
-    HIP_CHECK(hipStreamSynchronize(main_stream()));
+    sync_main();
   }
 
   void reshape(uint32_t w, uint32_t h, uint32_t r0, uint32_t n) {
-    HIP_CHECK(hipStreamSynchronize(main_stream()));
+    sync_main();
     sync_list_stream();
     release_buffers();
     W = w; H = h; row0 = r0; rows = n;
@@ -596,6 +608,8 @@
     bool have_lists = false;
     const bool build_lists = prepare_tile_lists(p, path, (flags & rtk::TRACE_ZERO_ACC) != 0u, have_lists);
     attach_sure_table(p, have_lists);
+    const bool from_idle = have_lists && lists_idle.exchange(false);
+    const bool list_wait = have_lists && (env.list_wait >= 0 ? env.list_wait != 0 : (build_lists && from_idle));
     last_k = K; last_chunk = p.chunk;
     last_lds = rtk::trace_lds_bytes(p, path == rtk::TracePath::DenseLists ? rtk::TracePath::ClassifyForms : path);
     const uint32_t r0 = allow_split ? split_row(p.rows) : 0u;
@@ -607,8 +621,8 @@
       (void)main_stream();
       if (build_lists) build_tile_lists_ahead(p);
       lists.attach(p, row0, have_lists);
+      if (list_wait) lists.wait(stream, 0);
       if (timed) HIP_CHECK(hipEventRecord(e.a, stream));
-      if (have_lists) lists.wait(stream, 0);
       attach_macro_lists(p, path, 0, stream, (flags & rtk::TRACE_ZERO_ACC) != 0u);
       HIP_CHECK(rtk::launch_trace(p, fma, filter, path, K, stream));
       if (timed) HIP_CHECK(hipEventRecord(e.b, stream));
@@ -626,10 +640,10 @@
       rtk::TraceParams half[2] = {sub_band(p, 0u, r0), sub_band(p, r0, p.rows - r0)};
       if (interleave) { half[0] = p; half[1] = p; half[0].row_il = half[1].row_il = 1u; half[1].row_phase = 1u; }
       hipStream_t st[2] = {stream, stream_b};
+      if (list_wait) { lists.wait(stream, 0); lists.wait(stream_b, 1); }
       if (timed) HIP_CHECK(hipEventRecord(e.a, stream));
       for (int h = 0; h < 2; ++h) {
         lists.attach(half[h], row0, have_lists);
-        if (have_lists) lists.wait(st[h], h);
         if (h == 1 && stagger) {
           const uint32_t us = static_cast<uint32_t>(clock.last_half_ms() * 450.0f);
           if (us >= 5u) HIP_CHECK(rtk::launch_delay(us, stream_b));
@@ -683,12 +697,15 @@
   void fetch_image() {
     HIP_CHECK(hipMemcpyAsync(h_image.get(), d_image.get(), static_cast<size_t>(npix()) * sizeof(uint32_t),
                              hipMemcpyDeviceToHost, main_stream()));
-    HIP_CHECK(hipStreamSynchronize(main_stream()));
+    sync_main();
   }
 
   rtr::TileListRing lists;
+  rtr::DevArray<unsigned long long> d_list_fallbacks;
   rtr::Event stagger_event;
   std::atomic<bool> stagger_next{true};
+  std::atomic<bool> lists_idle{true};
+  void sync_main() { HIP_CHECK(hipStreamSynchronize(main_stream())); lists_idle = true; }
   rtr::DevArray<uint32_t> d_half_cost;
   rtr::PinnedArray<unsigned long long> h_half_cost;
   bool rows_interleaved = false;
@@ -709,7 +726,7 @@
     const uint64_t seen = clock.seq_now();
     HIP_CHECK(hipStreamSynchronize(main_stream()));
     sync_list_stream();
-    stagger_next = true;
+    stagger_next = true; lists_idle = true;
     clock.drain_before(seen);
   }
   uint32_t scene_generation = 0;
@@ -729,7 +746,7 @@
     if (!have) return false;
     const size_t tiles = static_cast<size_t>((W + 31u) / 32u) * ((rows + 7u) / 8u + 1u) * 4u;
     return lists.prepare(tiles * (1u + p.bin_list), make_key(p, p.bin_list), !(first_launch_of_trace && !reuse_across_traces),
-                         [&] { HIP_CHECK(hipStreamSynchronize(main_stream())); });
+                         [&] { sync_main(); });
   }
 
   rtr::DevArray<float4> d_sure_table;
@@ -754,6 +771,7 @@
     const uint64_t m = lists.build_ahead();
     rtk::TraceParams q = p_band;
     lists.attach(q, row0, true);
+    q.list_tag = lists.tag(); q.list_fallbacks = nullptr;
     const uint32_t sr = split_row(rows);
     if (sr != 0u && d_half_cost.get() != nullptr && env.row_interleave < 0 && (m % 32u) == 0u) { q.half_cost = d_half_cost.get(); q.cost_split_brow = sr / 8u; }
     HIP_CHECK(rtk::launch_tile_lists(q, fma, stream_l));
@@ -767,6 +785,7 @@
     (void)prepare_tile_lists(p, path, true, have_lists);
     sync_list_stream();
     lists.attach(p, row0, have_lists);
+    p.list_tag = lists.tag_in_stream(); p.list_fallbacks = nullptr;
     if (have_lists) HIP_CHECK(rtk::launch_tile_lists(p, fma, main_stream()));
     attach_macro_lists(p, path, 0, main_stream());
     {
@@ -774,7 +793,7 @@
       take_uniform_state(p);
       HIP_CHECK(rtk::launch_trace(p, fma, filter, path, pick_k(samples), main_stream()));
     }
-    HIP_CHECK(hipStreamSynchronize(main_stream()));
+    sync_main();
   }
 
   rtr::HalfLists half_lists[2];
@@ -913,9 +932,10 @@
         clear_accumulators();
         if (!stopped) convert();
       }
-      if (stopped) { HIP_CHECK(hipStreamSynchronize(main_stream())); return; }
+      if (stopped) { sync_main(); return; }
       if (cleared && i == iterationCount) {
         sync_polling(main_stream());
+        lists_idle = true;
       } else {
         fetch_image();
         final_image = h_image.get();
```

Result: slower. 411,300 (-31.3%).
